# LIS-TU-Berlin/SVN-ICP

Measured on AMD Instinct MI355X. Metric: scan-pair registrations/sec at N particles x M source pts, 1/2/4/8 GPU, higher is better.
Workload: dtype f64; 1 GPU; C3: 128 particles SVN-ICP, 131072-pt source vs 262144-pt target, K=100, I=20, max_dist=1.0, lr=1.0, SVNFullGrad=False, correspondence=fast, early stop off; synthetic 64-beam scans (seed 20250718); particles=128, target_points=262144, knn_count=100, parallelism=single GPU

## Files before the change

### __graft_entry__.py

```python
from __future__ import annotations

import importlib.util
import os
import subprocess
import sys

ROOT = os.path.dirname(os.path.abspath(__file__))
PKG_DIR = os.path.join(ROOT, "svn-icp_amd")


def load_package():
    if "svnicp_amd" in sys.modules:
        return sys.modules["svnicp_amd"]
    spec = importlib.util.spec_from_file_location("svnicp_amd", os.path.join(PKG_DIR, "__init__.py"),
                                                  submodule_search_locations=[PKG_DIR])
    mod = importlib.util.module_from_spec(spec)
    sys.modules["svnicp_amd"] = mod
    spec.loader.exec_module(mod)
    return mod


def load_oracle():
    if "oracle_py" in sys.modules:
        return sys.modules["oracle_py"]
    spec = importlib.util.spec_from_file_location("oracle_py", os.path.join(ROOT, "oracle", "oracle_py.py"))
    mod = importlib.util.module_from_spec(spec)
    sys.modules["oracle_py"] = mod
    spec.loader.exec_module(mod)
    return mod


def build() -> None:
    jobs = str(min(4, os.cpu_count() or 1))
    subprocess.check_call(["make", "-C", os.path.join(PKG_DIR, "csrc"), "-j", jobs])
    subprocess.check_call(["make", "-C", os.path.join(ROOT, "oracle"), "libsvnicp_oracle.so"])
    subprocess.check_call(["make", "-C", os.path.join(ROOT, "tests", "microbench")])
    if os.path.isdir("/root/reference"):
        subprocess.check_call(["make", "-C", os.path.join(ROOT, "oracle"), "ref"])
    build_cpp_host()
    pkg = load_package()
    pkg.load_library()


def build_cpp_host() -> str:
    host = os.path.join(PKG_DIR, "host")
    exe = os.path.join(host, "sharded_drive")
    srcs = [os.path.join(host, f) for f in ("sharded_drive.cpp", "sharded_registration.hpp", "svnicp_hip_shim.hpp")]
    srcs.append(os.path.join(PKG_DIR, "libsvnicp_hip.so"))
    if os.path.exists(exe) and all(os.path.getmtime(exe) >= os.path.getmtime(f) for f in srcs):
        return exe
    subprocess.check_call(["/opt/rocm/bin/hipcc", "-std=c++17", "-O2", "-Wall", "-Werror", "-I", os.path.join(ROOT, "include"), "-I", host,
                           os.path.join(host, "sharded_drive.cpp"), "-L", PKG_DIR, "-lsvnicp_hip", "-lrccl",
                           "-Wl,-rpath,$ORIGIN/..", "-o", exe])
    return exe


def smoke() -> None:
    import numpy as np
    pkg = load_package()
    orc = load_oracle()
    P, B, M, K, I = 8, 512, 2048, 16, 6
    src, tgt = pkg.scans.random_clouds(B, M, seed=3)
    init = pkg.scans.make_particles(P, seed=3) * 0.2
    prm = pkg.SteinICPParam(iterations=I, lr=1.0, max_dist=1.0, KNN_count=K, SVN_full_grad=False)
    s = pkg.SVNICP(prm, init, pkg.ParticleWeightOpt())
    s.add_cloud(src, tgt, init)
    s.set_initial_mean(np.eye(4))
    assert s.stein_align() == pkg.SteinICPState.ALIGN_SUCCESS
    o = orc.Solver(init, iterations=I, lr=1.0, max_dist=1.0, knn_count=K, svn_full_grad=False)
    o.add_cloud(src, tgt, init)
    o.stein_align()
    assert np.array_equal(s.get_candidates().astype(np.int64), o.candidates()), "stage-A indices differ from oracle"
    err = np.abs(s.get_transformation() - o.get_transformation()).max()
    assert err < 1e-4, f"pose differs from oracle by {err}"
    print(f"smoke ok: pose {s.get_transformation()}  |hip - oracle|max = {err:.3e}")


if __name__ == "__main__":
    build()
    if len(sys.argv) > 1 and sys.argv[1] == "smoke":
        smoke()
```

### svn-icp_amd/csrc/api.hip

```cpp
#include "../../include/svnicp_hip.h"

#include <cmath>
#include <algorithm>
#include <cstdio>
#include <cstdlib>
#include <cstring>
#include <string>
#include <vector>

#include "device_buffer.hpp"
#include "kernels.hpp"
#include "stage_a_host.hpp"
#include "stage_b_host.hpp"

using namespace svnicp;
using namespace svnicp_host;

namespace {

struct CloudState {
  DevBuf<double> src, tgt;
  bool src_set = false, tgt_set = false;
};

struct SteinState {
  DevBuf<double> init_pose, R, t, Rtot, pose_out, eul, opt, uctl, work, stats;
  DevBuf<float> history;
  DevBuf<int> ctl;
  int hist_I = 0, hist_P = 0;
  PinnedBuf<double> h_init, h_stats;
  bool host_stats_valid = false;
  Event ev_init;
  bool init_in_flight = false;
  StepPlan step;
  DrivePlan drive;
  int single_done_it = -1;
  Event ev_fork, ev_join;
  bool median_pending = false;
  DevBuf<unsigned int> small_bar;
  bool small_launched = false;
  Event ev_chunk[3];
  PinnedBuf<int> h_flags;
  bool finish_seen = true;
  int finish_iter = 0;
};

struct Sharding {
  int p_lo = 0, p_hi = 0;
  bool set = false;
  int row_rank = 0, row_world = 1;
  int64_t B_total = 0;
  DevBuf<double> rank_sums;
};

struct MiniBatch {
  int batch = 0;
  uint64_t seed = 0, n = 0;
  bool explicit_tab = false;
  int tab_I = 0;
  std::vector<int32_t> tab_h;
  int64_t tab_checked_B = -1;
  bool on = false, have = false;
  bool check = false;
  int64_t rows = 0, nq = 0;
  unsigned long long base = 0;
  DevBuf<int32_t> tab, idx, flag, pos, bsum, cand;
  DevBuf<int> ctl;
  DevBuf<double> src_u, src;
};

struct PlaneState {
  int residual = SVNICP_RESIDUAL_POINT;
  double delta = 0.1;
  int normal_k = 16;
  bool supplied = false;
  bool estimated = false;
  int est_k = 0;
  int64_t passes = 0;
  bool on = false;
  DevBuf<double> rec;
  DevBuf<double> nsup;
  DevBuf<int32_t> nbr;
  DevBuf<double> nbr_d2;
  DevBuf<double> partial, Hb, stats;
};

struct EvalState {
  DevBuf<double> q, d2, partial, result;
  DevBuf<int32_t> idx;
  PinnedBuf<double> h_result;
  bool have = false;
  int64_t rows = 0;
};

struct ScoreState {
  int kind = SVNICP_WEIGHT_UNIFORM;
  double gate = 0.0, temperature = 0.0;
  bool on = false;
  const char* reg_refusal = nullptr;
  DevBuf<double> partial, scores, poses, w;
  bool have = false;
  int P = 0;
};

struct Trace { DevBuf<double> H, b, N, phi, h; DevBuf<int32_t> corr; };

struct Profiling {
  Event ev[3];
  bool on = false;
  unsigned mask = 0;
  int pcur = -1;
  std::vector<Event> pev;
  std::vector<int> pcls;
  size_t pused = 0;
};

struct DebugCounters {
  DevBuf<unsigned long long> upd;
};

struct Progress {
  bool particles_set = false, began = false, have_candidates = false, have_result = false;
  bool table_built = false;
  bool d2_due = false;
};

}

struct svnicp_ctx {
  svnicp_params prm{};
  int device = 0, num_cus = 256;
  Stream own_stream, side;
  hipStream_t stream = nullptr;
  std::string err;
  static std::string& create_error() { thread_local std::string s; return s; }

  int64_t B = 0, M = 0;
  int K = 0, P = 0;
  Pose0 pose0{};
  Tuning tune{};
  CloudState cloud; StageA sa; StageB sb; SteinState st;
  Sharding shard; MiniBatch mb; PlaneState pl; EvalState ev; ScoreState sc;
  Trace tr; Profiling prof; DebugCounters dbg; Progress run;
};

enum { KC_KNN = 0, KC_TABLE = 1, KC_SEARCH = 2, KC_ACCUM = 3, KC_REDUCE = 4, KC_UPDATE = 5, KC_COUNT = SVNICP_KERNEL_CLASSES };

static hipError_t prof_begin(svnicp_ctx* c, int cls) {
  c->prof.pcur = -1;
  if (!c->prof.on || !((c->prof.mask >> cls) & 1u)) return hipSuccess;
  c->prof.pcur = cls;
  if (c->prof.pused * 2 + 2 > c->prof.pev.size()) {
    for (int i = 0; i < 2; ++i) {
      Event e;
      hipError_t r = e.create();
      if (r != hipSuccess) return r;
      c->prof.pev.push_back(std::move(e));
    }
    c->prof.pcls.push_back(cls);
  }
  c->prof.pcls[c->prof.pused] = cls;
  return hipEventRecord(c->prof.pev[2 * c->prof.pused], c->stream);
}
static hipError_t prof_end(svnicp_ctx* c) {
  if (!c->prof.on || c->prof.pcur < 0) return hipSuccess;
  c->prof.pcur = -1;
  hipError_t r = hipEventRecord(c->prof.pev[2 * c->prof.pused + 1], c->stream);
  c->prof.pused += 1;
  return r;
}

#define CTX_CHECK(ctx) do { if (!(ctx)) return SVNICP_ERR_INVALID; } while (0)

static int bind(svnicp_ctx* c) {
  HIPCHK(c, hipSetDevice(c->device));
  return 0;
}

static StageAEnv stage_a_env(const svnicp_ctx* c) {
  return {c->stream, c->tune, c->num_cus, c->prm.record_trace != 0, c->cloud.tgt.p, c->B, c->M, c->pose0};
}

static RegistrationFacts registration_facts(const svnicp_ctx* c, bool plane) {
  RegistrationFacts f;
  f.P = c->P; f.K = c->K; f.I = c->prm.iterations; f.B = c->B; f.M = c->M;
  f.svgd = c->prm.mode == SVNICP_MODE_SVGD; f.check_early_stop = c->prm.check_early_stop != 0; f.record_trace = c->prm.record_trace != 0;
  f.profiling = c->prof.on;
  f.shard_set = c->shard.set; f.p_lo = c->shard.p_lo; f.p_hi = c->shard.p_hi; f.row_world = c->shard.row_world;
  f.batch = c->mb.batch; f.explicit_tab = c->mb.explicit_tab; f.tab_I = c->mb.tab_I;
  f.plane = plane; f.normals_supplied = c->pl.supplied; f.normal_k = c->pl.normal_k;
  f.weighting = c->sc.kind;
  return f;
}

extern "C" {

int svnicp_abi_version(void) { return SVNICP_ABI_VERSION; }

const char* svnicp_last_error(const svnicp_ctx* ctx) { return ctx ? ctx->err.c_str() : svnicp_ctx::create_error().c_str(); }

int svnicp_create(const svnicp_params* params, int device, const double* init_pose6xP, int P, svnicp_ctx** out) {
  if (!params || !out) return fail<svnicp_ctx>(nullptr, SVNICP_ERR_INVALID, "svnicp_create: null argument");
  if (params->struct_size != (int32_t)sizeof(svnicp_params))
    return fail<svnicp_ctx>(nullptr, SVNICP_ERR_INVALID, "svnicp_create: svnicp_params.struct_size mismatch");
  if (params->iterations < 0 || params->knn_count < 1)
    return fail<svnicp_ctx>(nullptr, SVNICP_ERR_INVALID, "svnicp_create: iterations >= 0 and knn_count >= 1 required");
  if (params->mode != SVNICP_MODE_SVN && params->mode != SVNICP_MODE_SVGD)
    return fail<svnicp_ctx>(nullptr, SVNICP_ERR_INVALID, "svnicp_create: unknown mode");
  int ndev = 0;
  if (hipGetDeviceCount(&ndev) != hipSuccess || ndev <= 0)
    return fail<svnicp_ctx>(nullptr, SVNICP_ERR_NO_DEVICE, "svnicp_create: no HIP device visible (this library has no CPU path)");
  if (device < 0 || device >= ndev) return fail<svnicp_ctx>(nullptr, SVNICP_ERR_INVALID, "svnicp_create: bad device ordinal");
  hipDeviceProp_t prop;
  if (hipSetDevice(device) != hipSuccess || hipGetDeviceProperties(&prop, device) != hipSuccess)
    return fail<svnicp_ctx>(nullptr, SVNICP_ERR_HIP, "svnicp_create: hipGetDeviceProperties failed");
  if (std::strncmp(prop.gcnArchName, "gfx950", 6) != 0)
    return fail<svnicp_ctx>(nullptr, SVNICP_ERR_NO_DEVICE,
                std::string("svnicp_create: device is ") + prop.gcnArchName + ", this library carries gfx950 code only");
  svnicp_ctx* c = new svnicp_ctx();
  c->prm = *params;
  c->device = device;
  c->num_cus = prop.multiProcessorCount > 0 ? prop.multiProcessorCount : 256;
  c->K = params->knn_count;
  c->st.finish_iter = params->iterations;
  const double I3[9] = {1, 0, 0, 0, 1, 0, 0, 0, 1};
  std::memcpy(c->pose0.R0, I3, sizeof I3);
  c->pose0.t0[0] = c->pose0.t0[1] = c->pose0.t0[2] = 0.0;
  if (c->own_stream.create(hipStreamNonBlocking) != hipSuccess) { delete c; return fail<svnicp_ctx>(nullptr, SVNICP_ERR_HIP, "svnicp_create: hipStreamCreate failed"); }
  if (c->side.create(hipStreamNonBlocking) != hipSuccess ||
      c->st.ev_fork.create(hipEventDisableTiming) != hipSuccess || c->st.ev_join.create(hipEventDisableTiming) != hipSuccess ||
      c->st.ev_init.create(hipEventDisableTiming) != hipSuccess) {
    delete c;
    return fail<svnicp_ctx>(nullptr, SVNICP_ERR_HIP, "svnicp_create: hipStreamCreate / hipEventCreate failed");
  }
  c->stream = c->own_stream;
  for (auto& e : c->prof.ev)
    if (e.create() != hipSuccess) { delete c; return fail<svnicp_ctx>(nullptr, SVNICP_ERR_HIP, "hipEventCreate failed"); }
  if (c->st.ctl.ensure(4) != hipSuccess) { delete c; return fail<svnicp_ctx>(nullptr, SVNICP_ERR_NOMEM, "hipMalloc failed"); }
  *out = c;
  if (const char* e = getenv("SVNICP_OPTIONS")) {
    std::string all(e);
    size_t pos = 0;
    while (pos < all.size()) {
      const size_t end = all.find(';', pos) == std::string::npos ? all.size() : all.find(';', pos);
      const std::string kv = all.substr(pos, end - pos);
      const size_t eq = kv.find('=');
      if (eq != std::string::npos && svnicp_set_option(c, kv.substr(0, eq).c_str(), kv.substr(eq + 1).c_str()) != 0) {
        svnicp_ctx::create_error() = c->err; svnicp_destroy(c); *out = nullptr; return SVNICP_ERR_INVALID;
      }
      pos = end + 1;
    }
  }
  if (init_pose6xP) {
    int rc = svnicp_set_particles(c, init_pose6xP, P);
    if (rc != 0) { svnicp_ctx::create_error() = c->err; svnicp_destroy(c); *out = nullptr; return rc; }
  }
  return SVNICP_OK;
}

void svnicp_destroy(svnicp_ctx* c) {
  if (!c) return;
  (void)hipSetDevice(c->device);
  if (c->stream) (void)hipStreamSynchronize(c->stream);
  if (c->side) (void)hipStreamSynchronize(c->side);
  delete c;
}

int svnicp_set_stream(svnicp_ctx* c, void* hip_stream) {
  CTX_CHECK(c);
  if (bind(c)) return SVNICP_ERR_HIP;
  HIPCHK(c, hipStreamSynchronize(c->stream));
  c->stream = hip_stream == SVNICP_OWN_STREAM ? c->own_stream : reinterpret_cast<hipStream_t>(hip_stream);
  return SVNICP_OK;
}

static int check_small_kernel(svnicp_ctx* c);
static int check_minibatch_table(svnicp_ctx* c);
int svnicp_synchronize(svnicp_ctx* c) {
  CTX_CHECK(c);
  if (bind(c)) return SVNICP_ERR_HIP;
  HIPCHK(c, hipStreamSynchronize(c->stream));
  if (const int rc = check_small_kernel(c)) return rc;
  if (const int rc = check_minibatch_table(c)) return rc;
  if (c->run.have_result && c->st.h_stats.p) c->st.host_stats_valid = true;
  return SVNICP_OK;
}

static int upload_cloud(svnicp_ctx* c, DevBuf<double>& buf, const double* xyz, int64_t n, int mem_kind) {
  if (bind(c)) return SVNICP_ERR_HIP;
  HIPCHK(c, buf.ensure((size_t)n * 3));
  const hipMemcpyKind kind = mem_kind == SVNICP_MEM_DEVICE ? hipMemcpyDeviceToDevice : hipMemcpyHostToDevice;
  HIPCHK(c, hipMemcpyAsync(buf.p, xyz, (size_t)n * 24, kind, c->stream));
  if (mem_kind != SVNICP_MEM_DEVICE) HIPCHK(c, hipStreamSynchronize(c->stream));
  c->run.have_candidates = false;
  return SVNICP_OK;
}

int svnicp_set_source(svnicp_ctx* c, const double* src, int64_t B, int mem_kind) {
  CTX_CHECK(c);
  if (!src || B < 1) return fail(c, SVNICP_ERR_INVALID, "svnicp_set_source: need B >= 1");
  if (B > 0x7fffffffLL) return fail(c, SVNICP_ERR_INVALID, "svnicp_set_source: cloud too large");
  if (const int rc = upload_cloud(c, c->cloud.src, src, B, mem_kind)) return rc;
  c->B = B;
  c->cloud.src_set = true;
  return SVNICP_OK;
}

int svnicp_set_target(svnicp_ctx* c, const double* tgt, int64_t M, int mem_kind) {
  CTX_CHECK(c);
  if (!tgt || M < 1) return fail(c, SVNICP_ERR_INVALID, "svnicp_set_target: need M >= 1");
  if (M > 0x7fffffffLL) return fail(c, SVNICP_ERR_INVALID, "svnicp_set_target: cloud too large");
  if (const int rc = upload_cloud(c, c->cloud.tgt, tgt, M, mem_kind)) return rc;
  c->M = M;
  c->sa.held = TargetLayout::None;
  c->cloud.tgt_set = true;
  c->pl.supplied = false; c->pl.estimated = false;
  return SVNICP_OK;
}

int svnicp_set_clouds(svnicp_ctx* c, const double* src, int64_t B, const double* tgt, int64_t M, int mem_kind) {
  CTX_CHECK(c);
  if (!src || !tgt || B < 1 || M < 1) return fail(c, SVNICP_ERR_INVALID, "svnicp_set_clouds: need B >= 1, M >= 1");
  if (M > 0x7fffffffLL || B > 0x7fffffffLL) return fail(c, SVNICP_ERR_INVALID, "svnicp_set_clouds: cloud too large");
  if (const int rc = svnicp_set_source(c, src, B, mem_kind)) return rc;
  return svnicp_set_target(c, tgt, M, mem_kind);
}

int svnicp_set_particles(svnicp_ctx* c, const double* init, int P) {
  CTX_CHECK(c);
  if (!init || P < 1) return fail(c, SVNICP_ERR_INVALID, "svnicp_set_particles: need P >= 1");
  if (bind(c)) return SVNICP_ERR_HIP;
  HIPCHK(c, c->st.init_pose.ensure((size_t)P * 6));
  HIPCHK(c, c->st.R.ensure((size_t)P * 9));
  HIPCHK(c, c->st.t.ensure((size_t)P * 3));
  HIPCHK(c, c->st.Rtot.ensure((size_t)P * 12));
  HIPCHK(c, c->st.pose_out.ensure((size_t)P * 6));
  HIPCHK(c, c->sb.sums.ensure((size_t)P * kNSums));
  HIPCHK(c, c->st.stats.ensure((size_t)48 + P));
  HIPCHK(c, c->st.work.ensure(update_workspace_doubles(P)));
  HIPCHK(c, c->st.eul.ensure((size_t)P * 6));
  HIPCHK(c, c->st.opt.ensure((size_t)P * 18));
  HIPCHK(c, c->st.uctl.ensure(update_uctl_doubles(P)));
  if ((size_t)P * 6 > c->st.h_init.cap || (size_t)P + 48 > c->st.h_stats.cap) {
    HIPCHK(c, hipStreamSynchronize(c->stream));
    HIPCHK(c, c->st.h_init.alloc((size_t)P * 6));
    HIPCHK(c, c->st.h_stats.alloc((size_t)P + 48));
  } else if (c->st.init_in_flight) {
    HIPCHK(c, hipEventSynchronize(c->st.ev_init));
  }
  std::memcpy(c->st.h_init.p, init, (size_t)P * 48);
  HIPCHK(c, hipMemcpyAsync(c->st.init_pose.p, c->st.h_init.p, (size_t)P * 48, hipMemcpyHostToDevice, c->stream));
  HIPCHK(c, hipEventRecord(c->st.ev_init, c->stream));
  c->st.init_in_flight = true;
  c->st.host_stats_valid = false;
  const bool first = !c->run.particles_set || P != c->P;
  if (P != c->P) c->sc.have = false;
  if (first && c->shard.row_world > 1) { c->shard.row_world = 1; c->shard.row_rank = 0; c->shard.B_total = 0; }
  c->P = P;
  if (!c->shard.set || first) { c->shard.p_lo = 0; c->shard.p_hi = P; c->shard.set = false; }
  HIPCHK(c, launch_init_particles(c->st.init_pose.p, P, c->pose0, c->prm.mode, c->st.R.p, c->st.t.p, c->st.Rtot.p, c->st.pose_out.p,
                                  (first || c->prm.mode == SVNICP_MODE_SVN) ? 1 : 0, c->st.eul.p, c->stream));
  c->run.particles_set = true;
  return SVNICP_OK;
}

int svnicp_set_initial_mean(svnicp_ctx* c, const double R0[9], const double t0[3]) {
  CTX_CHECK(c);
  if (!R0 || !t0) return fail(c, SVNICP_ERR_INVALID, "svnicp_set_initial_mean: null argument");
  std::memcpy(c->pose0.R0, R0, 9 * sizeof(double));
  std::memcpy(c->pose0.t0, t0, 3 * sizeof(double));
  c->run.have_candidates = false;
  return SVNICP_OK;
}

int svnicp_set_k(svnicp_ctx* c, int k) {
  CTX_CHECK(c);
  if (k < 1) return fail(c, SVNICP_ERR_INVALID, "svnicp_set_k: k >= 1 required");
  c->K = k;
  c->run.have_candidates = false;
  return SVNICP_OK;
}

int svnicp_set_max_dist(svnicp_ctx* c, double md) {
  CTX_CHECK(c);
  c->prm.max_dist = md;
  return SVNICP_OK;
}

int svnicp_set_option(svnicp_ctx* c, const char* name, const char* value) {
  CTX_CHECK(c);
  if (!name || !value) return fail(c, SVNICP_ERR_INVALID, "svnicp_set_option: null argument");
  const std::string k(name), v(value);
  Tuning& t = c->tune;
  auto num = [&](int lo, int hi, int* out) { char* end = nullptr; const long x = strtol(v.c_str(), &end, 10);
                                             if (end == v.c_str() || *end || x < lo || x > hi) return false; *out = (int)x; return true; };
  bool ok = true;
  if (k == "knn") { if (v == "auto") t.knn = {}; else if (v == "v1") t.knn = {false, KnnKernel::Stream}; else if (v == "v2") t.knn = {false, KnnKernel::SeededScan};
                    else if (v == "brute") t.knn = {false, KnnKernel::Brute}; else if (v == "tiles") t.knn = {false, KnnKernel::Tiles}; else ok = false; }
  else if (k == "knn_prefilter") { if (v == "mfma") t.knn_prefilter_mfma = 1; else if (v == "valu") t.knn_prefilter_mfma = 0; else ok = false; }
  else if (k == "fallback_sliced_max") ok = num(-1, 1 << 20, &t.fallback_sliced_max);
  else if (k == "accum") { if (v == "f64") t.accum = 0; else if (v == "valu") t.accum = 1; else if (v == "split") t.accum = 3; else ok = false; }
  else if (k == "update") { if (v == "auto") t.update_fused = 0; else if (v == "fused") t.update_fused = 1; else ok = false; }
  else if (k == "fused_update_max_p") ok = num(1, 700, &t.fused_update_max_p);
  else if (k == "wgpcu") { int x = 0, y = 0; ok = sscanf(v.c_str(), "%d,%d", &x, &y) == 2 && x >= 0 && x <= 64 && y >= 0 && y <= 16; if (ok) { t.wgpcu_search = x; t.wgpcu_accum = y; } }
  else if (k == "tp") ok = num(0, 1 << 16, &t.tp);
  else if (k == "debug") ok = num(0, 1, &t.debug);
  else if (k == "scan_split") ok = num(0, 16, &t.scan_split);
  else if (k == "group_stride") ok = num(0, 1 << 30, &t.group_stride);
  else if (k == "accum_min_steps") ok = num(0, 1 << 20, &t.accum_min_steps);
  else if (k == "brute_qb") { ok = num(0, 6, &t.brute_qb); }
  else if (k == "single") { if (v == "fused") t.single_fused = 1; else if (v == "split") t.single_fused = 0; else ok = false; }
  else if (k == "chain") { if (v == "auto") { t.small_chain = 1; t.persistent = 0; } else if (v == "persistent") { t.small_chain = 1; t.persistent = 1; }
                           else if (v == "general") { t.small_chain = 0; t.persistent = 0; } else ok = false; }
  else if (k == "median") { if (v == "auto") t.median_inline = -1; else if (v == "stream") t.median_inline = 0; else if (v == "inline") t.median_inline = 1; else ok = false; }
  else if (k == "sort") { if (v == "joint") t.sort_joint = 1; else if (v == "separate") t.sort_joint = 0; else ok = false; }
  else if (k == "table") { if (v == "select") t.table_select = 1; else if (v == "gather") t.table_select = 0; else ok = false; }
  else if (k == "correspondence") { if (v == "fast") t.full_corr = 0; else if (v == "full") t.full_corr = 1; else ok = false; }
  else return fail(c, SVNICP_ERR_INVALID, "svnicp_set_option: unknown option '" + k + "'");
  if (!ok) return fail(c, SVNICP_ERR_INVALID, "svnicp_set_option: bad value '" + v + "' for option '" + k + "'");
  c->run.have_candidates = false;
  c->sa.held = TargetLayout::None;
  if (c->run.began) c->st.step = plan_step(registration_facts(c, c->pl.on), c->tune, c->sb.plan);
  return SVNICP_OK;
}

int svnicp_set_shard(svnicp_ctx* c, int p_lo, int p_hi) {
  CTX_CHECK(c);
  if (!c->run.particles_set || p_lo < 0 || p_hi > c->P || p_lo > p_hi)
    return fail(c, SVNICP_ERR_INVALID, "svnicp_set_shard: need 0 <= p_lo <= p_hi <= P after svnicp_set_particles");
  c->shard.p_lo = p_lo; c->shard.p_hi = p_hi; c->shard.set = true;
  return SVNICP_OK;
}

int svnicp_set_row_shard(svnicp_ctx* c, int row_rank, int row_world, int64_t total_source_points) {
  CTX_CHECK(c);
  if (!c->run.particles_set || row_world < 1 || row_rank < 0 || row_rank >= row_world || (row_world > 1 && total_source_points < 1))
    return fail(c, SVNICP_ERR_INVALID, "svnicp_set_row_shard: need 0 <= row_rank < row_world and the whole scan's point count, after svnicp_set_particles");
  if (bind(c)) return SVNICP_ERR_HIP;
  c->shard.row_rank = row_rank; c->shard.row_world = row_world;
  c->shard.B_total = row_world > 1 ? total_source_points : 0;
  if (row_world > 1) {
    HIPCHK(c, c->shard.rank_sums.ensure((size_t)row_world * c->P * kNSums));
    HIPCHK(c, hipMemsetAsync(c->shard.rank_sums.p, 0, (size_t)row_world * c->P * kNSums * sizeof(double), c->stream));
  }
  return SVNICP_OK;
}

void* svnicp_rank_sums_devptr(svnicp_ctx* c) { return (c && c->shard.row_world > 1) ? (void*)c->shard.rank_sums.p : nullptr; }

static bool normal_pass_due(const svnicp_ctx* c) {
  return c->pl.on && !c->pl.supplied && !(c->pl.estimated && c->pl.est_k == c->pl.normal_k);
}

static int prepare_plane(svnicp_ctx* c);
int svnicp_align_begin(svnicp_ctx* c) {
  CTX_CHECK(c);
  if (!c->cloud.src_set || !c->cloud.tgt_set || !c->run.particles_set)
    return fail(c, SVNICP_ERR_INVALID, "svnicp_align: svnicp_set_clouds and svnicp_set_particles must come first");
  if (bind(c)) return SVNICP_ERR_HIP;
  const int I = c->prm.iterations, P = c->P;
  const int64_t B = c->B;
  const bool plane = c->pl.residual == SVNICP_RESIDUAL_PLANE;
  const RegistrationFacts f = registration_facts(c, plane);
  if (const char* why = minibatch_refusal(f, c->tune)) return fail(c, SVNICP_ERR_INVALID, std::string(kMinibatchRefusal) + why);
  if (c->mb.batch != 0 && c->mb.explicit_tab && !c->mb.tab_h.empty() && c->mb.tab_checked_B != B) {
    for (const int32_t v : c->mb.tab_h)
      if (v < 0 || (int64_t)v >= B)
        return fail(c, SVNICP_ERR_INVALID, "svnicp_align: the mini-batch index table holds " + std::to_string(v) + ", outside [0, " + std::to_string(B) + ")");
    c->mb.tab_checked_B = B;
  }
  if (const char* why = plane_refusal(f, c->tune)) return fail(c, SVNICP_ERR_INVALID, std::string(kPlaneRefusal) + why);
  if (const char* why = weighting_refusal(f, c->tune)) return fail(c, SVNICP_ERR_INVALID, std::string(kWeightingRefusal) + why);
  if (f.weighting && score_tile_rows(P, c->K, true) < 1)
    return fail(c, SVNICP_ERR_INVALID, std::string(kWeightingRefusal) + "knn_count is too large for one row's candidates to fit the scoring kernel's LDS tile");
  const RegistrationRows r = registration_rows(c->mb.batch, I, B);
  const AccumPlan shape = plan_stage_b(f, c->tune, r.Bi);
  const bool stage_a_k1 = StageA::plan_for(stage_a_env(c), r.Bq, c->K).can_search(1);
  if (const char* why = full_corr_refusal(f, c->tune, shape.f32, stage_a_k1)) return fail(c, SVNICP_ERR_INVALID, why);
  c->pl.on = plane;
  c->sc.on = f.weighting != 0; c->sc.reg_refusal = scoring_refusal(f, c->tune);
  c->mb.on = r.mb; c->mb.have = false; c->mb.check = false;
  c->mb.rows = r.mb ? r.Bt : 0;
  c->mb.nq = r.mb ? r.Bq : 0;
  HIPCHK(c, hipEventRecord(c->prof.ev[0], c->stream));
  const bool joint = joint_morton_sort(f, c->tune, StageA::plan_for(stage_a_env(c), r.Bq, c->K));
  if (const int rc = c->sa.begin(c, stage_a_env(c), r.Bq, c->K, {c->K, normal_pass_due(c) ? c->pl.normal_k : c->K, c->tune.full_corr ? 1 : c->K}, joint)) return rc;
  c->sa.writes_table = select_writes_table(f, c->tune, c->sa.plan, shape);
  c->run.table_built = false; c->run.d2_due = false;
  if (r.mb) {
    HIPCHK(c, c->mb.idx.ensure((size_t)r.Bt)); HIPCHK(c, c->mb.flag.ensure((size_t)B)); HIPCHK(c, c->mb.pos.ensure((size_t)B));
    HIPCHK(c, c->mb.bsum.ensure((size_t)minibatch_scan_blocks(B))); HIPCHK(c, c->mb.ctl.ensure(2));
    HIPCHK(c, c->mb.src_u.ensure((size_t)r.Bq * 3)); HIPCHK(c, c->mb.src.ensure((size_t)r.Bt * 3));
    HIPCHK(c, c->mb.cand.ensure((size_t)r.Bt * c->K));
  }
  if (const int rc = c->sb.begin(c, f, c->tune, r, shape, c->num_cus)) return rc;
  HIPCHK(c, c->st.history.ensure((size_t)(I > 0 ? I : 1) * 6 * P));
  c->st.hist_I = I; c->st.hist_P = P;
  if (c->prm.record_trace) {
    const size_t IP = (size_t)I * P;
    HIPCHK(c, c->tr.corr.ensure(IP * r.Bi));
    HIPCHK(c, hipMemsetAsync(c->tr.corr.p, 0xff, IP * r.Bi * 4, c->stream));
    const struct { DevBuf<double>& buf; size_t n; } dbl[] = {{c->tr.H, IP * 36}, {c->tr.b, IP * 6}, {c->tr.N, IP * 6}, {c->tr.phi, IP * 6}, {c->tr.h, (size_t)I + 1}};
    for (const auto& x : dbl) {
      HIPCHK(c, x.buf.ensure(x.n));
      HIPCHK(c, hipMemsetAsync(x.buf.p, 0, x.n * 8, c->stream));
    }
  }
  c->prof.pused = 0;
  c->st.single_done_it = -1;
  if (c->st.median_pending) HIPCHK(c, hipStreamWaitEvent(c->stream, c->st.ev_join, 0));
  c->st.median_pending = false;
  if (!c->st.finish_seen && c->prm.mode == SVNICP_MODE_SVGD && c->prm.check_early_stop) {
    int v[2] = {0, 0};
    HIPCHK(c, hipMemcpyAsync(v, c->st.ctl.p, sizeof v, hipMemcpyDeviceToHost, c->stream));
    HIPCHK(c, hipStreamSynchronize(c->stream));
    if (v[0]) c->st.finish_iter = v[1];
    c->st.finish_seen = true;
  }
  {
    BeginZero z{};
    auto add = [&](void* p, size_t bytes) { if (p && bytes) { z.ptr[z.n] = static_cast<unsigned int*>(p); z.dwords[z.n] = (unsigned int)(bytes / 4); ++z.n; } };
    add(c->st.uctl.p, update_uctl_doubles(P) * sizeof(double));
    add(c->st.history.p, (size_t)(I > 0 ? I : 1) * 6 * P * sizeof(float));
    add(c->sb.ambig.p, 2 * sizeof(int));
    if (c->sa.plan.kernel == KnnKernel::Brute) add(c->sa.fail_count.p, sizeof(int));
    HIPCHK(c, c->st.small_bar.ensure(8));
    add(c->st.small_bar.p, 8 * sizeof(unsigned int));
    if (c->prm.mode == SVNICP_MODE_SVGD) add(c->st.opt.p, (size_t)P * 18 * sizeof(double));
    z.ctl = c->st.ctl.p; z.iterations = I;
    HIPCHK(c, launch_init_particles(c->st.init_pose.p, P, c->pose0, 2, c->st.R.p, c->st.t.p, c->st.Rtot.p, c->st.pose_out.p, 0,
                                    nullptr, c->stream, &z));
  }
  if (c->mb.batch > 0 && !c->mb.explicit_tab) {
    c->mb.base = minibatch_stream_base(c->mb.seed, c->mb.n);
    c->mb.n += 1;
  }
  if (plane)
    if (const int rc = prepare_plane(c)) return rc;
  c->st.step = plan_step(f, c->tune, c->sb.plan);
  c->run.began = true;
  c->st.finish_seen = false;
  c->run.have_result = false;
  return SVNICP_OK;
}

static int ensure_dbg_upd(svnicp_ctx* c) {
  if (!c->tune.debug || c->dbg.upd.p) return SVNICP_OK;
  HIPCHK(c, c->dbg.upd.ensure(8));
  HIPCHK(c, hipMemset(c->dbg.upd.p, 0, 8 * sizeof(unsigned long long)));
  return SVNICP_OK;
}

static int print_update_phases(svnicp_ctx* c, bool persistent) {
  unsigned long long h[8];
  HIPCHK(c, hipStreamSynchronize(c->stream));
  if (!persistent) HIPCHK(c, hipStreamSynchronize(c->side));
  HIPCHK(c, hipMemcpy(h, c->dbg.upd.p, sizeof h, hipMemcpyDeviceToHost));
  if (persistent)
    fprintf(stderr, "[svnicp] k_small_registration, workgroup 0, cycles over %d iterations: search %llu | barrier %llu | accumulate %llu | barrier %llu | prepare %llu | barrier %llu | direction %llu | barrier %llu\n",
            c->prm.iterations, h[0], h[1], h[2], h[3], h[4], h[5], h[6], h[7]);
  else
    fprintf(stderr, "[svnicp] Stein step thread-0 cycles (summed over launches so far; fused kernel: prepare / median / direction / pose / tail; k_upd_median: state / histogram / bin scan / collect / rank): %llu %llu %llu %llu %llu\n", h[0], h[1], h[2], h[3], h[4]);
  return SVNICP_OK;
}

static int prepare_plane(svnicp_ctx* c) {
  HIPCHK(c, c->pl.partial.ensure((size_t)c->sb.plan.grid_x * c->sb.plan.Ppad * kPlaneSums));
  HIPCHK(c, c->pl.Hb.ensure((size_t)c->P * 42));
  HIPCHK(c, c->pl.stats.ensure((size_t)c->P * 2));
  HIPCHK(c, hipMemsetAsync(c->pl.stats.p, 0, (size_t)c->P * 2 * sizeof(double), c->stream));
  const int kn = c->pl.normal_k;
  if (!normal_pass_due(c)) return SVNICP_OK;
  if (!c->sa.plan.can_search(kn))
    return fail(c, SVNICP_ERR_INVALID, "svnicp_align: the seeded-scan stage A (option knn=v2, or a target beyond the tile kernel's range) cannot "
                                       "search with normal_k neighbours: supply the normals (svnicp_set_target_normals)");
  const int64_t M = c->M, rows = c->sa.block_rows(M);
  HIPCHK(c, c->pl.rec.ensure((size_t)M * 6));
  HIPCHK(c, c->pl.nbr.ensure((size_t)rows * kn));
  HIPCHK(c, c->pl.nbr_d2.ensure((size_t)rows * kn));
  const int rc = c->sa.search_blocks(c, stage_a_env(c), c->cloud.tgt.p, M, kn, c->pl.nbr.p, c->pl.nbr_d2.p, 0, [&](int64_t lo, int64_t n) {
    HIPCHK(c, launch_target_normals(c->cloud.tgt.p, M, c->pl.nbr.p, lo, n, kn, c->pl.rec.p, c->stream));
    return (int)SVNICP_OK;
  });
  if (rc) return rc;
  c->pl.estimated = true; c->pl.est_k = kn;
  c->pl.passes += 1;
  return SVNICP_OK;
}

int svnicp_stage_candidates(svnicp_ctx* c, int64_t b_lo, int64_t b_hi) {
  CTX_CHECK(c);
  if (!c->run.began) return fail(c, SVNICP_ERR_INVALID, "svnicp_stage_candidates: call svnicp_align_begin first");
  if (b_lo < 0 || b_hi > c->B || b_lo > b_hi) return fail(c, SVNICP_ERR_INVALID, "svnicp_stage_candidates: bad row range");
  if (bind(c)) return SVNICP_ERR_HIP;
  if (c->mb.on) {
    if (b_lo != 0 || b_hi != c->B)
      return fail(c, SVNICP_ERR_INVALID, "svnicp_stage_candidates: in mini-batch mode only the whole range (0, B) is accepted");
    MinibatchArgs m{};
    m.explicit_idx = c->mb.explicit_tab ? c->mb.tab.p : nullptr; m.idx = c->mb.idx.p; m.n = c->mb.rows; m.B = c->B; m.base = c->mb.base;
    m.flag = c->mb.flag.p; m.pos = c->mb.pos.p; m.block_sums = c->mb.bsum.p; m.mbctl = c->mb.ctl.p; m.ctl = c->st.ctl.p;
    m.src = c->cloud.src.p; m.src_u = c->mb.src_u.p; m.n_q = c->mb.nq;
    HIPCHK(c, prof_begin(c, KC_KNN));
    HIPCHK(c, launch_minibatch_draw_compact(m, c->stream));
    const int rc = c->sa.search(c, stage_a_env(c), c->mb.src_u.p, c->pose0, c->K, c->sa.cand_idx.p, c->sa.cand_d2.p, 0, c->mb.nq);
    if (rc) return rc;
    HIPCHK(c, launch_minibatch_expand(m, c->sa.cand_idx.p, c->K, c->mb.src.p, c->mb.cand.p, c->stream));
    HIPCHK(c, prof_end(c));
    c->mb.have = true;
    c->mb.check = c->mb.explicit_tab && c->mb.tab_h.empty();
    return SVNICP_OK;
  }
  HIPCHK(c, prof_begin(c, KC_KNN));
  const bool whole = b_lo == 0 && b_hi == c->B;
  const bool hand_over = c->sa.writes_table && whole;
  const TableOut tbl{c->sb.tablea.p, c->sb.anchor.p, c->sb.cmaxb.p};
  if (const int rc = c->sa.search(c, stage_a_env(c), c->cloud.src.p, c->pose0, c->K, c->sa.cand_idx.p, c->sa.cand_d2.p, b_lo, b_hi,
                                  hand_over ? &tbl : nullptr, whole)) return rc;
  c->run.table_built = hand_over; c->run.d2_due = hand_over;
  if (c->tune.full_corr)
    if (const int rc = c->sa.keep_stage_fallbacks(c, stage_a_env(c))) return rc;
  HIPCHK(c, prof_end(c));
  return SVNICP_OK;
}


int svnicp_build_candidate_table(svnicp_ctx* c) {
  CTX_CHECK(c);
  if (!c->run.began) return fail(c, SVNICP_ERR_INVALID, "svnicp_build_candidate_table: call svnicp_align_begin first");
  if (bind(c)) return SVNICP_ERR_HIP;
  if (c->mb.on && !c->mb.have) return fail(c, SVNICP_ERR_INVALID, "svnicp_build_candidate_table: call svnicp_stage_candidates(0, B) first");
  HIPCHK(c, prof_begin(c, KC_TABLE));
  const int32_t* cand = c->mb.on ? c->mb.cand.p : c->sa.cand_idx.p;
  const int64_t rows = c->mb.on ? c->mb.rows : c->B;
  if (!c->run.table_built)
    if (const int rc = c->sb.build_table(c, cand, rows, c->K, c->cloud.tgt.p, c->M, c->stream)) return rc;
  HIPCHK(c, prof_end(c));
  HIPCHK(c, hipEventRecord(c->prof.ev[1], c->stream));
  c->run.have_candidates = true;
  return SVNICP_OK;
}

static UpdateArgs update_args(svnicp_ctx* c, int it) {
  UpdateArgs u{};
  u.sums = c->shard.row_world > 1 ? c->shard.rank_sums.p : c->sb.sums.p; u.n_ranks = c->shard.row_world; u.R = c->st.R.p; u.t = c->st.t.p; u.Rtot = c->st.Rtot.p; u.pose = c->pose0;
  u.P = c->P; u.iteration = it; u.iterations = c->prm.iterations;
  u.lr = c->prm.lr; u.conv_thr = c->prm.convergence_threshold;
  u.check_early_stop = c->prm.check_early_stop; u.full_grad = c->prm.svn_full_grad;
  u.work = c->st.work.p; u.history = c->st.history.p; u.pose_out = c->st.pose_out.p; u.ctl = c->st.ctl.p;
  if (c->prm.record_trace) {
    u.trH = c->tr.H.p + (size_t)it * c->P * 36; u.trb = c->tr.b.p + (size_t)it * c->P * 6;
    u.trN = c->tr.N.p + (size_t)it * c->P * 6; u.trphi = c->tr.phi.p + (size_t)it * c->P * 6; u.trh = c->tr.h.p + it;
  }
  u.eul = c->st.eul.p; u.opt = c->st.opt.p; u.optimizer = c->prm.optimizer;
  u.n_src = (double)(c->shard.row_world > 1 ? c->shard.B_total : c->B);
  u.uctl = c->st.uctl.p;
  u.dbg = c->tune.debug ? c->dbg.upd.p : nullptr;
  u.svgd = c->prm.mode == SVNICP_MODE_SVGD ? 1 : 0;
  u.plane_Hb = c->pl.on ? c->pl.Hb.p : nullptr;
  return u;
}
static AccumArgs accum_args(svnicp_ctx* c, int it) {
  AccumArgs a{};
  a.src = c->cloud.src.p; a.table = c->sb.table.p; a.tablef = c->sb.tablef.p; a.tablea = c->sb.tablea.p; a.kbest = c->sb.kbest.p; a.kidx = c->sb.kidx.p; a.tgt = c->cloud.tgt.p; a.cand = c->sa.cand_idx.p; a.anchor = c->sb.anchor.p; a.M = c->M; a.cmax = c->sb.cmaxb.p; a.ambig_count = c->sb.ambig.p;
  a.Rtot = c->st.Rtot.p; a.B = c->B; a.K = c->K;
  a.p_lo = c->shard.p_lo; a.p_hi = c->shard.p_hi; a.max_dist = c->prm.max_dist; a.partial = c->sb.partial.p; a.ctl = c->st.ctl.p;
  a.corr = c->prm.record_trace ? c->tr.corr.p + (size_t)it * c->P * c->B : nullptr;
  if (c->mb.on) {
    const size_t r0 = (size_t)it * c->mb.batch;
    a.src = c->mb.src.p + 3 * r0; a.cand = c->mb.cand.p + r0 * c->K; a.cmax = c->sb.cmaxb.p + r0; a.B = c->mb.batch;
    if (c->sb.table.p) a.table = c->sb.table.p + r0 * c->K * 3;
    if (c->sb.tablef.p) a.tablef = c->sb.tablef.p + r0 * c->K;
    if (c->sb.tablea.p) a.tablea = c->sb.tablea.p + r0 * 128;
    if (c->sb.anchor.p) a.anchor = c->sb.anchor.p + 3 * r0;
    if (c->prm.record_trace) a.corr = c->tr.corr.p + (size_t)it * c->P * c->mb.batch;
  }
  a.svgd = c->prm.mode == SVNICP_MODE_SVGD ? 1 : 0;
  a.fin_iteration = -1;
  if (c->st.drive.defer_fin && it >= 1) {
    const UpdateArgs up = update_args(c, it - 1);
    a.fin_iteration = it - 1; a.fin_P = c->P; a.fin_thr = c->prm.convergence_threshold; a.fin_norms = update_step_norms(up);
    a.fin_pose = c->st.pose_out.p; a.fin_history = c->st.history.p; a.fin_ctl = c->st.ctl.p;
  }
  a.ticket = reinterpret_cast<unsigned int*>(c->st.uctl.p + 41);
  return a;
}

static bool step_finishes(const svnicp_ctx* c, int it) { return !(c->st.drive.defer_fin && it < c->prm.iterations - 1); }

static int fork_median(svnicp_ctx* c, int it) {
  if (c->st.step.chain != StepChain::SideStream || c->st.median_pending) return SVNICP_OK;
  if (const int rc = ensure_dbg_upd(c)) return rc;
  const UpdateArgs u = update_args(c, it);
  HIPCHK(c, hipEventRecord(c->st.ev_fork, c->stream));
  HIPCHK(c, hipStreamWaitEvent(c->side, c->st.ev_fork, 0));
  HIPCHK(c, launch_update_median(u, c->num_cus, c->tune.fused_update_max_p, c->side));
  HIPCHK(c, hipEventRecord(c->st.ev_join, c->side));
  c->st.median_pending = true;
  return SVNICP_OK;
}

int svnicp_iter_accumulate(svnicp_ctx* c, int it) {
  CTX_CHECK(c);
  if (!c->run.began || !c->run.have_candidates)
    return fail(c, SVNICP_ERR_INVALID, "svnicp_iter_accumulate: candidates not staged");
  if (it < 0 || it >= c->prm.iterations) return fail(c, SVNICP_ERR_INVALID, "svnicp_iter_accumulate: bad iteration");
  if (bind(c)) return SVNICP_ERR_HIP;
  if (const int rc = fork_median(c, it)) return rc;
  const int nshard = c->shard.p_hi - c->shard.p_lo;
  if (nshard <= 0) return SVNICP_OK;
  AccumArgs a = accum_args(c, it);
  if (c->tune.full_corr) {
    HIPCHK(c, prof_begin(c, KC_SEARCH));
    for (int p = c->shard.p_lo; p < c->shard.p_hi; ++p) {
      HIPCHK(c, launch_transform_cloud(c->cloud.src.p, c->B, c->st.Rtot.p + 12 * (size_t)p, c->sb.full_q.p, c->st.ctl.p, c->stream));
      if (const int rc = c->sa.search_blocks(c, stage_a_env(c), c->sb.full_q.p, c->B, 1, c->sb.full_idx.p + (size_t)p * c->B, c->sb.full_d2.p, 1)) return rc;
    }
    HIPCHK(c, prof_end(c));
    a.full_idx = c->sb.full_idx.p;
  } else if (c->sb.plan.f32 == 3) {
    HIPCHK(c, prof_begin(c, KC_SEARCH));
    HIPCHK(c, launch_search_split(c->sb.plan, a, c->stream));
    HIPCHK(c, prof_end(c));
  }
  if (c->pl.on) {
    PlaneArgs pa{};
    pa.src = c->cloud.src.p; pa.rec = c->pl.rec.p; pa.Rtot = c->st.Rtot.p; pa.B = c->B; pa.M = c->M; pa.p_lo = c->shard.p_lo; pa.p_hi = c->shard.p_hi;
    pa.max_dist = c->prm.max_dist; pa.delta = c->pl.delta; pa.partial = c->pl.partial.p; pa.ctl = c->st.ctl.p;
    pa.kidx = c->sb.kidx.p; pa.kbest = c->sb.kbest.p; pa.corr = a.corr;
    HIPCHK(c, prof_begin(c, KC_ACCUM));
    HIPCHK(c, launch_plane_accumulate(c->sb.plan, pa, c->stream));
    HIPCHK(c, prof_end(c));
    HIPCHK(c, prof_begin(c, KC_REDUCE));
    HIPCHK(c, launch_plane_finalize(c->pl.partial.p, c->sb.plan.grid_x, c->sb.plan.Ppad, c->shard.p_lo, nshard, c->pl.Hb.p, c->pl.stats.p,
                                    c->st.ctl.p, c->stream));
    HIPCHK(c, prof_end(c));
    return SVNICP_OK;
  }
  const bool single = c->st.step.single_fused;
  const UpdateArgs us = update_args(c, it);
  HIPCHK(c, prof_begin(c, KC_ACCUM));
  HIPCHK(c, launch_accumulate(c->sb.plan, a, single ? &us : nullptr, c->stream));
  HIPCHK(c, prof_end(c));
  if (single) { c->st.single_done_it = it; return SVNICP_OK; }
  if (c->st.step.chain == StepChain::SmallChain) return SVNICP_OK;
  HIPCHK(c, prof_begin(c, KC_REDUCE));
  double* rec = c->shard.row_world > 1 ? c->shard.rank_sums.p + (size_t)c->shard.row_rank * c->P * kNSums : c->sb.sums.p;
  HIPCHK(c, launch_reduce_partials(c->sb.partial.p, c->sb.plan.grid_x, c->sb.plan.Ppad, c->shard.p_lo, nshard, rec, c->st.ctl.p, c->stream));
  HIPCHK(c, prof_end(c));
  return SVNICP_OK;
}

int svnicp_iter_update(svnicp_ctx* c, int it) {
  CTX_CHECK(c);
  if (!c->run.began) return fail(c, SVNICP_ERR_INVALID, "svnicp_iter_update: call svnicp_align_begin first");
  if (it < 0 || it >= c->prm.iterations) return fail(c, SVNICP_ERR_INVALID, "svnicp_iter_update: bad iteration");
  if (bind(c)) return SVNICP_ERR_HIP;
  if (c->st.single_done_it == it) { c->st.single_done_it = -1; return SVNICP_OK; }
  if (const int rc = ensure_dbg_upd(c)) return rc;
  UpdateArgs u = update_args(c, it);
  HIPCHK(c, prof_begin(c, KC_UPDATE));
  if (c->tune.debug && it == c->prm.iterations - 1)
    if (const int rc = print_update_phases(c, false)) return rc;
  const StepChain chain = c->st.step.chain;
  if (chain == StepChain::OneKernel) {
    u.svgd = 0;
    if (c->prm.mode == SVNICP_MODE_SVGD) HIPCHK(c, launch_update_svgd(u, c->stream));
    else HIPCHK(c, launch_update(u, c->stream));
  } else {
    if (chain == StepChain::SmallChain) {
      u.sums = c->sb.partial.p; u.n_ranks = c->sb.plan.grid_x; u.sums_stride = c->sb.plan.Ppad * kNSums; u.sums_out = c->sb.sums.p;
    }
    if (chain == StepChain::SideStream) {
      if (const int rc = fork_median(c, it)) return rc;
      HIPCHK(c, launch_update_prepare(u, c->stream));
      HIPCHK(c, hipStreamWaitEvent(c->stream, c->st.ev_join, 0));
      c->st.median_pending = false;
    } else {
      HIPCHK(c, launch_update_prepare_median(u, c->stream));
    }
    HIPCHK(c, launch_update_direction(u, c->stream, step_finishes(c, it)));
  }
  HIPCHK(c, prof_end(c));
  return SVNICP_OK;
}

static int enqueue_scoring(svnicp_ctx* c, double gate) {
  const bool normals = c->pl.supplied || c->pl.estimated;
  if (score_tile_rows(c->P, c->K, normals) < 1)
    return fail(c, SVNICP_ERR_INVALID, std::string(kScoringRefusal) + "knn_count is too large for one row's candidates to fit the scoring kernel's LDS tile");
  ScoreState& sc = c->sc;
  sc.have = false;
  HIPCHK(c, sc.partial.ensure((size_t)score_blocks(c->B) * score_padded_particles(c->P, c->K) * kScoreRecord));
  HIPCHK(c, sc.scores.ensure((size_t)c->P * kScoreFields));
  HIPCHK(c, sc.poses.ensure((size_t)c->P * 12));
  ScoreArgs a{};
  a.src = c->cloud.src.p; a.tgt = c->cloud.tgt.p; a.rec = normals ? c->pl.rec.p : nullptr; a.cand = c->sa.cand_idx.p; a.Rtot = c->st.Rtot.p;
  a.B = c->B; a.M = c->M; a.K = c->K; a.P = c->P; a.thr2 = gate * gate; a.partial = sc.partial.p;
  HIPCHK(c, launch_particle_score(a, sc.scores.p, c->stream));
  HIPCHK(c, hipMemcpyAsync(sc.poses.p, c->st.Rtot.p, (size_t)c->P * 12 * sizeof(double), hipMemcpyDeviceToDevice, c->stream));
  sc.have = true; sc.P = c->P;
  return SVNICP_OK;
}

int svnicp_finish(svnicp_ctx* c) {
  CTX_CHECK(c);
  if (!c->run.began) return fail(c, SVNICP_ERR_INVALID, "svnicp_finish: call svnicp_align_begin first");
  if (bind(c)) return SVNICP_ERR_HIP;
  HIPCHK(c, hipEventRecord(c->prof.ev[2], c->stream));
  StatsArgs s{c->st.pose_out.p, c->P, c->prm.mode, c->st.stats.p};
  if (c->sc.on) {
    if (const int rc = enqueue_scoring(c, c->sc.gate)) return rc;
    HIPCHK(c, c->sc.w.ensure((size_t)c->P));
    HIPCHK(c, launch_particle_weights(c->sc.scores.p, c->P, c->sc.temperature, c->sc.w.p, c->stream));
    HIPCHK(c, launch_stats_weighted(s, c->sc.w.p, c->stream));
  } else {
    HIPCHK(c, launch_stats(s, c->stream));
  }
  c->st.host_stats_valid = false;
  if (c->st.h_stats.p && (size_t)c->P + 48 <= c->st.h_stats.cap)
    HIPCHK(c, hipMemcpyAsync(c->st.h_stats.p, c->st.stats.p, ((size_t)c->P + 48) * 8, hipMemcpyDeviceToHost, c->stream));
  c->run.have_result = true;
  return SVNICP_OK;
}

int svnicp_stopped(svnicp_ctx* c) {
  CTX_CHECK(c);
  if (bind(c)) return SVNICP_ERR_HIP;
  int v[2] = {0, 0};
  HIPCHK(c, hipMemcpyAsync(v, c->st.ctl.p, sizeof v, hipMemcpyDeviceToHost, c->stream));
  HIPCHK(c, hipStreamSynchronize(c->stream));
  return v[0] ? 1 : 0;
}

void* svnicp_candidates_devptr(svnicp_ctx* c) { return c ? (void*)c->sa.cand_idx.p : nullptr; }
void* svnicp_sums_devptr(svnicp_ctx* c) { return c ? (void*)c->sb.sums.p : nullptr; }
void* svnicp_total_pose_devptr(svnicp_ctx* c) { return c ? (void*)c->st.Rtot.p : nullptr; }

static int align_enqueue(svnicp_ctx* c, bool follow_stop) {
  CTX_CHECK(c);
  if (c->prm.mode == SVNICP_MODE_SVGD && (c->prm.optimizer < 0 || c->prm.optimizer > 3))
    return SVNICP_NO_OPTIMIZER;
  int rc = svnicp_align_begin(c);
  if (rc) return rc;
  if ((rc = svnicp_stage_candidates(c, 0, c->B))) return rc;
  if ((rc = svnicp_build_candidate_table(c))) return rc;
  c->st.small_launched = false;
  const DrivePlan drive = plan_drive(registration_facts(c, c->pl.on), c->tune, c->sb.plan, c->st.step, follow_stop);
  c->st.drive = drive;
  c->st.drive.defer_fin = false;
  if (drive.persistent_try) {
    const AccumArgs a = accum_args(c, 0);
    if ((rc = ensure_dbg_upd(c))) return rc;
    if (c->tune.debug) HIPCHK(c, hipMemsetAsync(c->dbg.upd.p, 0, 8 * sizeof(unsigned long long), c->stream));
    UpdateArgs u = update_args(c, 0);
    u.sums_out = c->sb.sums.p;
    const hipError_t e = launch_small_registration(c->sb.plan, a, u, c->prm.iterations, c->st.small_bar.p, c->num_cus, c->stream);
    if (e == hipSuccess && c->tune.debug)
      if ((rc = print_update_phases(c, true))) return rc;
    if (e == hipSuccess) { c->st.small_launched = true; return svnicp_finish(c); }
    (void)hipGetLastError();
  }
  c->st.drive.defer_fin = drive.defer_fin;
  struct Reset { bool& f; ~Reset() { f = false; } } reset_defer{c->st.drive.defer_fin};
  if (drive.follow && !c->st.h_flags.p) {
    HIPCHK(c, c->st.h_flags.alloc(3));
    for (auto& e : c->st.ev_chunk) HIPCHK(c, e.create(hipEventDisableTiming));
  }
  for (int it = 0; it < c->prm.iterations; ++it) {
    if ((rc = svnicp_iter_accumulate(c, it))) return rc;
    if ((rc = svnicp_iter_update(c, it))) return rc;
    if (drive.follow && (it + 1) % kChunk == 0) {
      const int chunk = it / kChunk, slot = chunk % 3;
      HIPCHK(c, hipMemcpyAsync(&c->st.h_flags.p[slot], c->st.ctl.p, sizeof(int), hipMemcpyDeviceToHost, c->stream));
      HIPCHK(c, hipEventRecord(c->st.ev_chunk[slot], c->stream));
      if (chunk >= 1) {
        const int prev = (chunk - 1) % 3;
        HIPCHK(c, hipEventSynchronize(c->st.ev_chunk[prev]));
        if (c->st.h_flags.p[prev]) break;
      }
    }
  }
  return svnicp_finish(c);
}
int svnicp_align_async(svnicp_ctx* c) { return align_enqueue(c, false); }

static int check_small_kernel(svnicp_ctx* c) {
  if (!c->st.small_launched) return SVNICP_OK;
  c->st.small_launched = false;
  unsigned int w[2] = {0u, 0u};
  HIPCHK(c, hipMemcpyAsync(w, c->st.small_bar.p, sizeof w, hipMemcpyDeviceToHost, c->stream));
  HIPCHK(c, hipStreamSynchronize(c->stream));
  if (w[1] != 0u) { c->run.have_result = false; return fail(c, SVNICP_ERR_HIP, "svnicp_align: the small-registration kernel's grid barrier timed out (chain=persistent is an option; the default launches do not wait on each other)"); }
  return SVNICP_OK;
}

static int check_minibatch_table(svnicp_ctx* c) {
  if (!c->mb.check) return SVNICP_OK;
  c->mb.check = false;
  int w[2] = {0, 0};
  HIPCHK(c, hipMemcpyAsync(w, c->mb.ctl.p, sizeof w, hipMemcpyDeviceToHost, c->stream));
  HIPCHK(c, hipStreamSynchronize(c->stream));
  if (w[0]) {
    c->run.have_result = false; c->st.finish_seen = true;
    return fail(c, SVNICP_ERR_INVALID, "svnicp_align: the mini-batch index table holds a value outside [0, B); the registration did not run");
  }
  return SVNICP_OK;
}

int svnicp_align(svnicp_ctx* c) {
  CTX_CHECK(c);
  if (c->shard.set && (c->shard.p_lo != 0 || c->shard.p_hi != c->P))
    return fail(c, SVNICP_ERR_INVALID, "svnicp_align: a particle shard is set; drive the split-phase calls instead");
  if (c->shard.row_world > 1)
    return fail(c, SVNICP_ERR_INVALID, "svnicp_align: a source-row shard is set (this context holds a partial record); drive the split-phase calls instead");
  int rc = align_enqueue(c, true);
  if (rc) return rc;
  HIPCHK(c, hipStreamSynchronize(c->stream));
  if ((rc = check_small_kernel(c))) return rc;
  if ((rc = check_minibatch_table(c))) return rc;
  c->st.host_stats_valid = c->st.h_stats.p != nullptr;
  return SVNICP_ALIGN_SUCCESS;
}

static int fetch(svnicp_ctx* c, void* dst, const void* src, size_t bytes) {
  if (bind(c)) return SVNICP_ERR_HIP;
  HIPCHK(c, hipMemcpyAsync(dst, src, bytes, hipMemcpyDeviceToHost, c->stream));
  HIPCHK(c, hipStreamSynchronize(c->stream));
  return SVNICP_OK;
}
#define NEED_RESULT(c)                                                                   \
  do {                                                                                   \
    CTX_CHECK(c);                                                                        \
    if (!(c)->run.have_result) return fail((c), SVNICP_ERR_INVALID, "no registration result yet"); \
  } while (0)

static int fetch_stats(svnicp_ctx* c, void* dst, size_t off_doubles, size_t n_doubles) {
  if (c->st.host_stats_valid) { std::memcpy(dst, c->st.h_stats.p + off_doubles, n_doubles * 8); return SVNICP_OK; }
  return fetch(c, dst, c->st.stats.p + off_doubles, n_doubles * 8);
}
int svnicp_get_transformation(svnicp_ctx* c, double out6[6]) { NEED_RESULT(c); return fetch_stats(c, out6, 0, 6); }
int svnicp_get_distribution(svnicp_ctx* c, double out6[6]) { NEED_RESULT(c); return fetch_stats(c, out6, 6, 6); }
int svnicp_get_cov_matrix(svnicp_ctx* c, double out36[36]) { NEED_RESULT(c); return fetch_stats(c, out36, 12, 36); }
int svnicp_get_particle_weight(svnicp_ctx* c, double* outP) {
  NEED_RESULT(c);
  return fetch_stats(c, outP, 48, (size_t)c->P);
}
int svnicp_get_particles(svnicp_ctx* c, double* out6P) {
  CTX_CHECK(c);
  if (!c->run.particles_set) return fail(c, SVNICP_ERR_INVALID, "no particles set");
  return fetch(c, out6P, c->st.pose_out.p, (size_t)c->P * 48);
}
int svnicp_get_particle_history(svnicp_ctx* c, float* out) {
  NEED_RESULT(c);
  return fetch(c, out, c->st.history.p, (size_t)c->st.hist_I * 6 * c->st.hist_P * sizeof(float));
}

int svnicp_get_gpu_ms(svnicp_ctx* c, double out3[3]) {
  NEED_RESULT(c);
  if (bind(c)) return SVNICP_ERR_HIP;
  HIPCHK(c, hipStreamSynchronize(c->stream));
  float a = 0, b = 0;
  HIPCHK(c, hipEventElapsedTime(&a, c->prof.ev[0], c->prof.ev[1]));
  HIPCHK(c, hipEventElapsedTime(&b, c->prof.ev[1], c->prof.ev[2]));
  out3[0] = a; out3[1] = b; out3[2] = (double)a + b;
  return SVNICP_OK;
}

int svnicp_get_runtime(svnicp_ctx* c, double out3[3]) {
  NEED_RESULT(c);
  double ms[3];
  int rc = svnicp_get_gpu_ms(c, ms);
  if (rc) return rc;
  if (c->prm.mode == SVNICP_MODE_SVGD && c->prm.check_early_stop && !c->st.finish_seen) {
    int v[2] = {0, 0};
    HIPCHK(c, hipMemcpy(v, c->st.ctl.p, sizeof v, hipMemcpyDeviceToHost));
    if (v[0]) c->st.finish_iter = v[1];
    c->st.finish_seen = true;
  }
  out3[0] = ms[0] * 1e-3; out3[1] = ms[1] * 1e-3; out3[2] = (double)c->st.finish_iter;
  return SVNICP_OK;
}

int svnicp_get_iterations_run(svnicp_ctx* c, int* out) {
  NEED_RESULT(c);
  if (!out) return SVNICP_ERR_INVALID;
  int v[2];
  const int rc = fetch(c, v, c->st.ctl.p, sizeof v);
  if (rc) return rc;
  *out = v[1];
  return SVNICP_OK;
}

int svnicp_get_knn_fallbacks(svnicp_ctx* c, int* out) {
  CTX_CHECK(c);
  if (!c->run.have_candidates) return fail(c, SVNICP_ERR_INVALID, "no candidates yet");
  const int* count = c->sa.fallback_count();
  if (!count) { *out = -1; return SVNICP_OK; }
  return fetch(c, out, count, sizeof(int));
}

int svnicp_get_knn_fallback_rows(svnicp_ctx* c, int32_t* out, int cap, int* n_out) {
  CTX_CHECK(c);
  if (!c->run.have_candidates || !n_out) return fail(c, SVNICP_ERR_INVALID, "no candidates yet");
  *n_out = 0;
  const int* count = c->sa.fallback_count();
  if (!count) return SVNICP_OK;
  int n = 0;
  int rc = fetch(c, &n, count, sizeof(int));
  if (rc) return rc;
  *n_out = n;
  if (n > cap) n = cap;
  if (n > 0 && out) return fetch(c, out, c->sa.fallback_rows(), (size_t)n * 4);
  return SVNICP_OK;
}

int svnicp_get_knn_survivors(svnicp_ctx* c, int32_t* outB) {
  CTX_CHECK(c);
  const int32_t* n = c->run.have_candidates ? c->sa.survivors(c->prm.record_trace != 0) : nullptr;
  if (!n) return fail(c, SVNICP_ERR_INVALID, "svnicp_get_knn_survivors: needs record_trace and the pruned stage-A kernel");
  return fetch(c, outB, n, (size_t)c->B * 4);
}

int svnicp_get_ambiguous_steps(svnicp_ctx* c, int* out) {
  NEED_RESULT(c);
  if (c->sb.plan.f32 == 0) { *out = -1; return SVNICP_OK; }
  return fetch(c, out, c->sb.ambig.p, sizeof(int));
}

int svnicp_get_ambiguous_pairs(svnicp_ctx* c, int64_t* out) {
  CTX_CHECK(c);
  if (!c->run.have_result || !out) return fail(c, SVNICP_ERR_INVALID, "no registration result yet");
  if (c->sb.plan.f32 != 3) { *out = -1; return SVNICP_OK; }
  int v[2] = {0, 0};
  const int rc = fetch(c, v, c->sb.ambig.p, sizeof v);
  *out = v[1];
  return rc;
}

int svnicp_set_profile(svnicp_ctx* c, int on) {
  CTX_CHECK(c);
  c->prof.on = on != 0;
  c->prof.mask = on == 1 ? ~0u : ((unsigned)on >> 1);
  return SVNICP_OK;
}

int svnicp_get_kernel_ms(svnicp_ctx* c, double* ms5, int32_t* launches5) {
  NEED_RESULT(c);
  if (!c->prof.on) return fail(c, SVNICP_ERR_INVALID, "svnicp_get_kernel_ms: profiling is off (svnicp_set_profile)");
  if (bind(c)) return SVNICP_ERR_HIP;
  HIPCHK(c, hipStreamSynchronize(c->stream));
  for (int i = 0; i < KC_COUNT; ++i) { ms5[i] = 0.0; launches5[i] = 0; }
  for (size_t i = 0; i < c->prof.pused; ++i) {
    float ms = 0;
    HIPCHK(c, hipEventElapsedTime(&ms, c->prof.pev[2 * i], c->prof.pev[2 * i + 1]));
    ms5[c->prof.pcls[i]] += ms;
    launches5[c->prof.pcls[i]] += 1;
  }
  return SVNICP_OK;
}

static const char* const kMbCandMsg = "mini-batch mode: stage A ran on the drawn rows only, use svnicp_get_minibatch_candidates";
int svnicp_get_candidates(svnicp_ctx* c, int32_t* out) {
  CTX_CHECK(c);
  if (!c->run.have_candidates) return fail(c, SVNICP_ERR_INVALID, "no candidates yet");
  if (c->mb.on) return fail(c, SVNICP_ERR_INVALID, std::string("svnicp_get_candidates: ") + kMbCandMsg);
  return fetch(c, out, c->sa.cand_idx.p, (size_t)c->B * c->K * 4);
}
int svnicp_get_candidate_dist2(svnicp_ctx* c, double* out) {
  CTX_CHECK(c);
  if (!c->run.have_candidates) return fail(c, SVNICP_ERR_INVALID, "no candidates yet");
  if (c->mb.on) return fail(c, SVNICP_ERR_INVALID, std::string("svnicp_get_candidate_dist2: ") + kMbCandMsg);
  if (c->run.d2_due) {
    if (bind(c)) return SVNICP_ERR_HIP;
    HIPCHK(c, launch_candidate_dist2(c->cloud.src.p, c->pose0, c->cloud.tgt.p, c->M, c->sa.cand_idx.p, c->B, c->K, c->sa.cand_d2.p, c->stream));
    c->run.d2_due = false;
  }
  return fetch(c, out, c->sa.cand_d2.p, (size_t)c->B * c->K * 8);
}

int svnicp_set_minibatch(svnicp_ctx* c, int batch_size, uint64_t seed) {
  CTX_CHECK(c);
  c->mb.batch = batch_size;
  c->mb.seed = seed; c->mb.n = 0;
  c->mb.explicit_tab = false; c->mb.tab_I = 0; c->mb.tab_h.clear(); c->mb.tab_checked_B = -1;
  c->run.have_candidates = false;
  return SVNICP_OK;
}

int svnicp_set_minibatch_indices(svnicp_ctx* c, const int32_t* idx, int iterations, int batch_size, int mem_kind) {
  CTX_CHECK(c);
  if (!idx || iterations < 1 || batch_size < 1)
    return fail(c, SVNICP_ERR_INVALID, "svnicp_set_minibatch_indices: need a table of iterations >= 1 rows of batch_size >= 1 indices");
  const int64_t n = (int64_t)iterations * batch_size;
  if (n > kMinibatchMaxRows) return fail(c, SVNICP_ERR_INVALID, "svnicp_set_minibatch_indices: iterations * batch_size exceeds 2^22 table rows");
  if (bind(c)) return SVNICP_ERR_HIP;
  HIPCHK(c, hipStreamSynchronize(c->stream));
  HIPCHK(c, c->mb.tab.ensure((size_t)n));
  c->mb.tab_h.clear();
  if (mem_kind == SVNICP_MEM_DEVICE) {
    HIPCHK(c, hipMemcpyAsync(c->mb.tab.p, idx, (size_t)n * 4, hipMemcpyDeviceToDevice, c->stream));
  } else {
    c->mb.tab_h.assign(idx, idx + n);
    HIPCHK(c, hipMemcpyAsync(c->mb.tab.p, c->mb.tab_h.data(), (size_t)n * 4, hipMemcpyHostToDevice, c->stream));
    HIPCHK(c, hipStreamSynchronize(c->stream));
  }
  c->mb.batch = batch_size; c->mb.explicit_tab = true; c->mb.tab_I = iterations; c->mb.tab_checked_B = -1;
  c->run.have_candidates = false;
  return SVNICP_OK;
}

#define NEED_MINIBATCH(c, what)                                                                                          \
  do {                                                                                                                   \
    CTX_CHECK(c);                                                                                                        \
    if (!(c)->mb.on || !(c)->mb.have) return fail((c), SVNICP_ERR_INVALID, what ": no registration in mini-batch mode yet"); \
  } while (0)
int svnicp_get_minibatch_indices(svnicp_ctx* c, int32_t* out) {
  NEED_MINIBATCH(c, "svnicp_get_minibatch_indices");
  return fetch(c, out, c->mb.idx.p, (size_t)c->mb.rows * 4);
}
int svnicp_get_minibatch_candidates(svnicp_ctx* c, int32_t* out) {
  NEED_MINIBATCH(c, "svnicp_get_minibatch_candidates");
  return fetch(c, out, c->mb.cand.p, (size_t)c->mb.rows * c->K * 4);
}
int svnicp_get_minibatch_rows(svnicp_ctx* c, int64_t out2[2]) {
  NEED_MINIBATCH(c, "svnicp_get_minibatch_rows");
  if (!out2) return SVNICP_ERR_INVALID;
  int w[2] = {0, 0};
  const int rc = fetch(c, w, c->mb.ctl.p, sizeof w);
  if (rc) return rc;
  out2[0] = w[1]; out2[1] = c->mb.nq;
  return SVNICP_OK;
}

int svnicp_set_residual(svnicp_ctx* c, int residual, double huber_delta, int normal_k) {
  CTX_CHECK(c);
  if (residual != SVNICP_RESIDUAL_POINT && residual != SVNICP_RESIDUAL_PLANE) return fail(c, SVNICP_ERR_INVALID, "svnicp_set_residual: unknown residual");
  if (!(huber_delta > 0.0)) return fail(c, SVNICP_ERR_INVALID, "svnicp_set_residual: huber_delta must be positive (+inf: no down-weighting)");
  if (normal_k != 0 && (normal_k < 4 || normal_k > 64)) return fail(c, SVNICP_ERR_INVALID, "svnicp_set_residual: normal_k must be 0 (= 16) or in 4..64");
  c->pl.residual = residual; c->pl.delta = huber_delta; c->pl.normal_k = normal_k ? normal_k : 16;
  c->run.have_candidates = false;
  return SVNICP_OK;
}

int svnicp_set_target_normals(svnicp_ctx* c, const double* n_xyz, int64_t M, int mem_kind) {
  CTX_CHECK(c);
  if (!n_xyz) return fail(c, SVNICP_ERR_INVALID, "svnicp_set_target_normals: null argument");
  if (!c->cloud.tgt_set || M != c->M)
    return fail(c, SVNICP_ERR_INVALID, "svnicp_set_target_normals: must follow the svnicp_set_target it belongs to, with the same point count");
  if (bind(c)) return SVNICP_ERR_HIP;
  HIPCHK(c, c->pl.nsup.ensure((size_t)M * 3));
  HIPCHK(c, c->pl.rec.ensure((size_t)M * 6));
  HIPCHK(c, hipMemcpyAsync(c->pl.nsup.p, n_xyz, (size_t)M * 24, mem_kind == SVNICP_MEM_DEVICE ? hipMemcpyDeviceToDevice : hipMemcpyHostToDevice, c->stream));
  HIPCHK(c, launch_pack_normals(c->cloud.tgt.p, c->pl.nsup.p, M, c->pl.rec.p, c->stream));
  if (mem_kind != SVNICP_MEM_DEVICE) HIPCHK(c, hipStreamSynchronize(c->stream));
  c->pl.supplied = true; c->pl.estimated = false;
  return SVNICP_OK;
}

int svnicp_get_target_normals(svnicp_ctx* c, double* outMx3) {
  CTX_CHECK(c);
  if (!outMx3) return fail(c, SVNICP_ERR_INVALID, "svnicp_get_target_normals: null argument");
  if (!c->pl.supplied && !c->pl.estimated) return fail(c, SVNICP_ERR_INVALID, "svnicp_get_target_normals: no normals supplied or estimated for this target yet");
  std::vector<double> rec((size_t)c->M * 6);
  if (const int rc = fetch(c, rec.data(), c->pl.rec.p, rec.size() * 8)) return rc;
  for (int64_t i = 0; i < c->M; ++i)
    for (int d = 0; d < 3; ++d) outMx3[3 * i + d] = rec[6 * i + 3 + d];
  return SVNICP_OK;
}

int svnicp_get_plane_stats(svnicp_ctx* c, double* outPx2, int64_t* normal_passes) {
  CTX_CHECK(c);
  if (normal_passes) *normal_passes = c->pl.passes;
  if (!outPx2) return SVNICP_OK;
  if (!c->run.have_result || !c->pl.on) return fail(c, SVNICP_ERR_INVALID, "svnicp_get_plane_stats: no registration with the point-to-plane residual yet");
  return fetch(c, outPx2, c->pl.stats.p, (size_t)c->P * 16);
}

static void host_so3_exp(const double w[3], double R[9]) {
  const double th = std::sqrt(w[0] * w[0] + w[1] * w[1] + w[2] * w[2]);
  const double K[9] = {0, -w[2], w[1], w[2], 0, -w[0], -w[1], w[0], 0};
  double K2[9];
  for (int i = 0; i < 3; ++i)
    for (int j = 0; j < 3; ++j) K2[3 * i + j] = K[3 * i] * K[j] + K[3 * i + 1] * K[3 + j] + K[3 * i + 2] * K[6 + j];
  const double a = th < 1e-10 ? 1.0 : std::sin(th) / th, b = th < 1e-10 ? 0.5 : (1.0 - std::cos(th)) / (th * th);
  for (int i = 0; i < 9; ++i) R[i] = (i % 4 == 0 ? 1.0 : 0.0) + a * K[i] + b * K2[i];
}

int svnicp_evaluate(svnicp_ctx* c, const double* R, const double* t, double max_corr_dist, svnicp_eval* out) {
  CTX_CHECK(c);
  if (!out) return fail(c, SVNICP_ERR_INVALID, "svnicp_evaluate: null result struct");
  if (out->struct_size != (int32_t)sizeof(svnicp_eval)) return fail(c, SVNICP_ERR_INVALID, "svnicp_evaluate: svnicp_eval.struct_size mismatch");
  if (!(max_corr_dist > 0.0)) return fail(c, SVNICP_ERR_INVALID, "svnicp_evaluate: max_corr_dist must be positive and not NaN (+inf: every evaluated row with a finite distance is an inlier)");
  if ((R == nullptr) != (t == nullptr)) return fail(c, SVNICP_ERR_INVALID, "svnicp_evaluate: R and t must both be given, or both be NULL (the last registration's result)");
  if (R) {
    bool finite = true;
    for (int i = 0; i < 9; ++i) finite = finite && std::isfinite(R[i]);
    for (int i = 0; i < 3; ++i) finite = finite && std::isfinite(t[i]);
    if (!finite) return fail(c, SVNICP_ERR_INVALID, "svnicp_evaluate: the pose holds a non-finite entry");
  }
  if (!c->run.have_result)
    return fail(c, SVNICP_ERR_INVALID, "svnicp_evaluate: no finished registration yet (stage A's target layout and scratch belong to one)");
  if (!c->run.have_candidates)
    return fail(c, SVNICP_ERR_INVALID, "svnicp_evaluate: the source, the target, the initial mean, K or an option changed since the last registration: "
                                       "register again first (stage A's target layout and scratch belong to that registration)");
  if (!c->sa.plan.can_search(1))
    return fail(c, SVNICP_ERR_INVALID, "svnicp_evaluate: the seeded-scan stage A (option knn=v2, or a target beyond the tile kernel's range) is built "
                                       "for knn_count neighbours and cannot search with K = 1");
  if (const int rc = svnicp_synchronize(c)) return rc;
  EvalPose T{};
  if (R) {
    std::memcpy(T.R, R, sizeof T.R); std::memcpy(T.t, t, sizeof T.t);
  } else {
    double mean[6], Rc[9];
    if (const int rc = fetch_stats(c, mean, 0, 6)) return rc;
    host_so3_exp(mean + 3, Rc);
    const double* R0 = c->pose0.R0;
    for (int i = 0; i < 3; ++i) {
      for (int j = 0; j < 3; ++j) T.R[3 * i + j] = R0[3 * i] * Rc[j] + R0[3 * i + 1] * Rc[3 + j] + R0[3 * i + 2] * Rc[6 + j];
      T.t[i] = (R0[3 * i] * mean[0] + R0[3 * i + 1] * mean[1] + R0[3 * i + 2] * mean[2]) + c->pose0.t0[i];
    }
    for (int i = 0; i < 12; ++i)
      if (!std::isfinite(i < 9 ? T.R[i] : T.t[i - 9])) return fail(c, SVNICP_ERR_INVALID, "svnicp_evaluate: the last registration's result pose is not finite");
  }
  const int64_t B = c->B, M = c->M, nblk = evaluate_blocks(B);
  EvalState& ev = c->ev;
  ev.have = false;
  HIPCHK(c, ev.q.ensure((size_t)B * 3)); HIPCHK(c, ev.idx.ensure((size_t)B)); HIPCHK(c, ev.d2.ensure((size_t)B));
  HIPCHK(c, ev.partial.ensure((size_t)nblk * kEvalRecord)); HIPCHK(c, ev.result.ensure(kEvalResult));
  if (!ev.h_result.p) HIPCHK(c, ev.h_result.alloc(kEvalResult));
  HIPCHK(c, launch_evaluate_transform(c->cloud.src.p, B, T, ev.q.p, c->stream));
  const StageAEnv env{c->stream, c->tune, c->num_cus, false, c->cloud.tgt.p, c->B, c->M, c->pose0};
  if (!c->sa.stage_kept)
    if (const int rc = c->sa.keep_stage_fallbacks(c, env)) return rc;
  if (const int rc = c->sa.search_blocks(c, env, ev.q.p, B, 1, ev.idx.p, ev.d2.p, 1)) return rc;
  const bool normals = c->pl.supplied || c->pl.estimated;
  EvalArgs a{};
  a.q = ev.q.p; a.tgt = c->cloud.tgt.p; a.rec = normals ? c->pl.rec.p : nullptr; a.B = B; a.M = M;
  a.thr2 = max_corr_dist * max_corr_dist; a.idx = ev.idx.p; a.d2 = ev.d2.p; a.partial = ev.partial.p;
  HIPCHK(c, launch_evaluate_pairs(a, ev.result.p, c->stream));
  HIPCHK(c, hipMemcpyAsync(ev.h_result.p, ev.result.p, kEvalResult * sizeof(double), hipMemcpyDeviceToHost, c->stream));
  HIPCHK(c, hipStreamSynchronize(c->stream));
  const double* r = ev.h_result.p;
  out->has_normals = normals ? 1 : 0;
  out->rows = B;
  out->evaluated = (int64_t)r[0]; out->inliers = (int64_t)r[1]; out->plane_inliers = (int64_t)r[2];
  out->sum_d2 = r[3]; out->sum_r2 = r[4]; out->fitness = r[5]; out->inlier_rmse = r[6]; out->plane_rmse = r[7];
  std::memcpy(out->R, T.R, sizeof T.R); std::memcpy(out->t, T.t, sizeof T.t);
  ev.have = true; ev.rows = B;
  return SVNICP_OK;
}

const int32_t* svnicp_eval_index_devptr(svnicp_ctx* c) { return (c && c->ev.have) ? c->ev.idx.p : nullptr; }
const double* svnicp_eval_dist2_devptr(svnicp_ctx* c) { return (c && c->ev.have) ? c->ev.d2.p : nullptr; }

int svnicp_get_eval_pairs(svnicp_ctx* c, int32_t* idxB, double* d2B) {
  CTX_CHECK(c);
  if (!c->ev.have) return fail(c, SVNICP_ERR_INVALID, "svnicp_get_eval_pairs: no svnicp_evaluate yet");
  if (idxB)
    if (const int rc = fetch(c, idxB, c->ev.idx.p, (size_t)c->ev.rows * 4)) return rc;
  if (d2B)
    if (const int rc = fetch(c, d2B, c->ev.d2.p, (size_t)c->ev.rows * 8)) return rc;
  return SVNICP_OK;
}

int svnicp_get_particle_scores(svnicp_ctx* c, double* outPx6, double* posesPx12) {
  CTX_CHECK(c);
  if (!c->sc.have) return fail(c, SVNICP_ERR_INVALID, "svnicp_get_particle_scores: no scoring yet (svnicp_score_particles, or a registration with svnicp_set_particle_weighting)");
  if (outPx6)
    if (const int rc = fetch(c, outPx6, c->sc.scores.p, (size_t)c->sc.P * kScoreFields * sizeof(double))) return rc;
  if (posesPx12)
    if (const int rc = fetch(c, posesPx12, c->sc.poses.p, (size_t)c->sc.P * 12 * sizeof(double))) return rc;
  return SVNICP_OK;
}

int svnicp_score_particles(svnicp_ctx* c, double max_corr_dist, double* outPx6, double* posesPx12) {
  CTX_CHECK(c);
  if (!(max_corr_dist > 0.0) || !std::isfinite(max_corr_dist))
    return fail(c, SVNICP_ERR_INVALID, "svnicp_score_particles: max_corr_dist must be finite and positive");
  if (!c->run.have_result)
    return fail(c, SVNICP_ERR_INVALID, "svnicp_score_particles: no finished registration yet (the candidate table belongs to one)");
  if (!c->run.have_candidates)
    return fail(c, SVNICP_ERR_INVALID, "svnicp_score_particles: the source, the target, the initial mean, K or an option changed since the last registration: "
                                       "register again first (the candidate table belongs to that registration)");
  if (c->sc.reg_refusal) return fail(c, SVNICP_ERR_INVALID, std::string(kScoringRefusal) + c->sc.reg_refusal);
  if (const int rc = svnicp_synchronize(c)) return rc;
  if (bind(c)) return SVNICP_ERR_HIP;
  if (const int rc = enqueue_scoring(c, max_corr_dist)) return rc;
  if (!outPx6 && !posesPx12) { HIPCHK(c, hipStreamSynchronize(c->stream)); return SVNICP_OK; }
  return svnicp_get_particle_scores(c, outPx6, posesPx12);
}

int svnicp_set_particle_weighting(svnicp_ctx* c, int kind, double max_corr_dist, double temperature) {
  CTX_CHECK(c);
  if (kind != SVNICP_WEIGHT_UNIFORM) {
    if (!(max_corr_dist > 0.0) || !std::isfinite(max_corr_dist))
      return fail(c, SVNICP_ERR_INVALID, "svnicp_set_particle_weighting: max_corr_dist must be finite and positive");
    if (!(temperature > 0.0) || !std::isfinite(temperature))
      return fail(c, SVNICP_ERR_INVALID, "svnicp_set_particle_weighting: temperature must be finite and positive");
  }
  c->sc.kind = kind;
  c->sc.gate = max_corr_dist; c->sc.temperature = temperature;
  return SVNICP_OK;
}

int svnicp_get_trace(svnicp_ctx* c, int32_t* corr, double* H, double* b, double* N, double* phi, double* h) {
  NEED_RESULT(c);
  if (!c->prm.record_trace) return fail(c, SVNICP_ERR_INVALID, "svnicp_get_trace: params.record_trace was 0");
  const size_t I = (size_t)c->prm.iterations, P = (size_t)c->P;
  int rc = 0;
  if (corr && (rc = fetch(c, corr, c->tr.corr.p, I * P * (size_t)(c->mb.on ? c->mb.batch : c->B) * 4))) return rc;
  if (H && (rc = fetch(c, H, c->tr.H.p, I * P * 36 * 8))) return rc;
  if (b && (rc = fetch(c, b, c->tr.b.p, I * P * 6 * 8))) return rc;
  if (N && (rc = fetch(c, N, c->tr.N.p, I * P * 6 * 8))) return rc;
  if (phi && (rc = fetch(c, phi, c->tr.phi.p, I * P * 6 * 8))) return rc;
  if (h && (rc = fetch(c, h, c->tr.h.p, I * 8))) return rc;
  return SVNICP_OK;
}

}
```

### svn-icp_amd/csrc/kernels.hpp

```cpp
#pragma once
#include "device_math.hpp"
#include "registration_plan.hpp"
#include "stage_a_plan.hpp"

namespace svnicp {

struct KnnArgs {
  const double* src;
  Pose0 pose;
  const double *tx, *ty, *tz;
  const int32_t* torig;
  int64_t M, Mp;
  int64_t b_lo, b_hi;
  int K, S;
  double* pool_d;
  int32_t* pool_i;
  int32_t* out_idx;
  double* out_d2;
  const int32_t* qlist;
  const int* qlist_count;
  int list_grid;
  int list_qw;
  int slices, slice_max_queries, merge_n;
  double* sl_d;
  int32_t* sl_i;
  const double* qthr;
};
hipError_t launch_knn_merge_slices(const KnnArgs& a, hipStream_t st);

struct KnnBruteArgs {
  const double* src;
  Pose0 pose;
  const double* tgt;
  int64_t M;
  int64_t b_lo, b_hi;
  int K;
  int32_t* out_idx;
  double* out_d2;
  unsigned long long* phase_cycles;
};
int knn_brute_queries_per_block(int64_t n, int num_cus);
hipError_t launch_knn_brute(const KnnBruteArgs& a, int num_cus, int queries_per_block, hipStream_t st);

struct KnnScanArgs {
  const double* src;
  Pose0 pose;
  const double *tx, *ty, *tz;
  const float *txf, *tyf, *tzf;
  const int32_t* torig;
  const unsigned long long* emax_bits;
  int64_t M, Mp, Ms;
  int64_t b_lo, b_hi;
  int K, S2, seed_rank;
  int32_t* pool;
  int32_t* out_idx;
  double* out_d2;
  int32_t* fail_list;
  int* fail_count;
};
hipError_t launch_targets_soa2(const double* tgt, int64_t M, int64_t Mp, double* tx, double* ty, double* tz,
                               float* txf, float* tyf, float* tzf, int32_t* torig, unsigned long long* emax_bits,
                               hipStream_t st);
hipError_t launch_knn_scan(const KnnScanArgs& a, hipStream_t st);
hipError_t launch_knn_topk(const KnnArgs& a, hipStream_t st);

struct KnnTilesArgs {
  const double* src;
  Pose0 pose;
  const int32_t* qorder;
  const double *tx, *ty, *tz;
  const float *txf, *tyf, *tzf;
  const int32_t* torig;
  const float* tile_box;
  const unsigned long long* emax_bits;
  const float4* tile_a;
  const float4* tile_o;
  int prefilter_mfma;
  int64_t M, Mp;
  int n_tiles;
  int64_t b_lo, b_hi;
  int K, S2;
  int32_t* pool;
  int32_t* arena;
  int32_t* chunk_tab;
  int arena_cap;
  int64_t tab_rows;
  int scan_split;
  unsigned int group_stride;
  int32_t* out_idx;
  double* out_d2;
  const double* tgt;
  float4* tbl_a;
  double* tbl_anchor;
  float* tbl_cmax;
  int32_t* fail_list;
  int* fail_count;
  int32_t* stat_n;
  unsigned long long* phase_cycles;
  void* qrec;
  double* fail_tau;
};
hipError_t launch_knn_tiles(const KnnTilesArgs& a, hipStream_t st);
hipError_t launch_candidate_dist2(const double* src, const Pose0& pose, const double* tgt, int64_t M, const int32_t* idx, int64_t B, int K,
                                  double* d2, hipStream_t st);
size_t sort_temp_bytes(size_t n, int key_bits);
hipError_t launch_bbox(const double* pts, int64_t n, unsigned long long* bbox, hipStream_t st);
hipError_t launch_morton_order(const double* pts, int64_t i0, int64_t n, int transform, const Pose0& pose,
                               const unsigned long long* bbox, unsigned int* keys_a, unsigned int* keys_b,
                               int32_t* vals_a, int32_t* order, void* temp, size_t temp_bytes, hipStream_t st);
hipError_t launch_morton_order_joint(const double* tgt, int64_t M, const double* qsrc, int64_t n, const Pose0& pose,
                                     const unsigned long long* bbox, unsigned int* keys_a, unsigned int* keys_b,
                                     int32_t* vals_a, int32_t* order, void* temp, size_t temp_bytes, hipStream_t st);
hipError_t launch_targets_sorted(const double* tgt, int64_t M, int64_t Mp, const int32_t* order, double* tx, double* ty,
                                 double* tz, float* txf, float* tyf, float* tzf, int32_t* torig, float* tile_box,
                                 unsigned long long* emax_bits, float4* tile_a, float4* tile_o, hipStream_t st);

struct AccumArgs {
  const double* src;
  const double* table;
  const float4* tablef;
  const float4* tablea;
  const float* cmax;
  int* ambig_count;
  const double* Rtot;
  int64_t B;
  int K, RS;
  int p_lo, p_hi;
  int TP;
  int tiles_per_block;
  int64_t n_tiles;
  int Ppad;
  double max_dist;
  double* partial;
  const int* ctl;
  int32_t* corr;
  int svgd;
  const double* tgt;
  const int32_t* cand;
  const double* anchor;
  int64_t M;
  uint8_t* kbest;
  int32_t* kidx;
  const int32_t* full_idx;
  int pts_per_block, spts_per_block;
  unsigned int* ticket;
  int fin_iteration, fin_P;
  double fin_thr;
  const double* fin_norms;
  const double* fin_pose;
  float* fin_history;
  int* fin_ctl;
};
AccumPlan plan_accumulate(AccumPlan shape, int64_t B, int num_cus, const Tuning& tune);
hipError_t launch_search_split(const AccumPlan& plan, AccumArgs a, hipStream_t st);
hipError_t launch_accumulate_split(const AccumPlan& plan, const AccumArgs& a, hipStream_t st);
void split_occupancy_blocks(int PW, int WP, int K, size_t smem, int* search, int* accum);
hipError_t launch_build_table3(const int32_t* idx, int64_t B, int K, const double* tgt, int64_t M, double* table,
                               double* anchor, float4* tablea, float* cmax, hipStream_t st);
hipError_t launch_build_table3_list(const int32_t* idx, const int32_t* list, const int* count, int64_t B, int K, const double* tgt,
                                    int64_t M, double* anchor, float4* tablea, float* cmax, hipStream_t st);
hipError_t launch_build_table2(const int32_t* idx, int64_t B, int K, const double* tgt, int64_t M, double* table,
                               float4* tablef, float* cmax, hipStream_t st);
hipError_t launch_transform_cloud(const double* src, int64_t B, const double* pose12, double* q, const int* ctl, hipStream_t st);
struct UpdateArgs {
  const double* sums;
  int n_ranks;
  int sums_stride;
  double* sums_out;
  double* R;
  double* t;
  double* Rtot;
  Pose0 pose;
  int P, iteration, iterations;
  double lr, conv_thr;
  int check_early_stop, full_grad;
  double* work;
  float* history;
  double* pose_out;
  int* ctl;
  double *trH, *trb, *trN, *trphi, *trh;
  int h_in_lds;
  double* eul;
  double* opt;
  int svgd;
  int optimizer;
  double n_src;
  double* uctl;
  unsigned long long* dbg;
  const double* plane_Hb;
};
size_t update_workspace_doubles(int P);
struct BeginZero { unsigned int* ptr[6]; unsigned int dwords[6]; int n; int* ctl; int iterations; };
hipError_t launch_init_particles(const double* init6xP, int P, const Pose0& pose, int mode, double* R, double* t,
                                 double* Rtot, double* pose_out, int refresh_pose, double* eul, hipStream_t st, const BeginZero* zero = nullptr);
int single_particle_grid(int64_t B);
hipError_t launch_accumulate(const AccumPlan& plan, AccumArgs a, const UpdateArgs* single, hipStream_t st);
hipError_t launch_update_svgd(const UpdateArgs& a, hipStream_t st);
hipError_t launch_update(const UpdateArgs& a, hipStream_t st);
hipError_t launch_update_median(const UpdateArgs& a, int num_cus, int max_p_one_workgroup, hipStream_t st);
hipError_t launch_update_prepare(const UpdateArgs& a, hipStream_t st);
hipError_t launch_update_prepare_median(const UpdateArgs& a, hipStream_t st);
hipError_t launch_small_registration(const AccumPlan& plan, AccumArgs a, const UpdateArgs& u, int iterations, unsigned int* bar,
                                     int num_cus, hipStream_t st);
hipError_t launch_update_direction(const UpdateArgs& a, hipStream_t st, bool finish = true);
const double* update_step_norms(const UpdateArgs& a);
hipError_t launch_reduce_partials(const double* partial, int nblk, int Ppad, int p_lo, int n_particles, double* sums, const int* ctl,
                                  hipStream_t st);
size_t update_uctl_doubles(int P);
constexpr int kPlaneSums = 29;
constexpr double kPlaneMinRatio = 0.01;
struct PlaneArgs {
  const double* src;
  const double* rec;
  const double* Rtot;
  int64_t B, M;
  int p_lo, p_hi;
  int Ppad;
  int pts_per_block;
  double max_dist, delta;
  double* partial;
  const int* ctl;
  const int32_t* kidx;
  const uint8_t* kbest;
  int32_t* corr;
};
hipError_t launch_target_normals(const double* tgt, int64_t M, const int32_t* nbr, int64_t row_lo, int64_t rows, int kn, double* rec,
                                 hipStream_t st);
hipError_t launch_pack_normals(const double* tgt, const double* nrm, int64_t M, double* rec, hipStream_t st);
hipError_t launch_plane_accumulate(const AccumPlan& plan, PlaneArgs a, hipStream_t st);
hipError_t launch_plane_finalize(const double* partial, int nblk, int Ppad, int p_lo, int n_particles, double* Hb, double* stats,
                                 const int* ctl, hipStream_t st);
constexpr int kEvalRecord = 5;
constexpr int kEvalResult = 8;
struct EvalPose { double R[9]; double t[3]; };
struct EvalArgs {
  const double* q;
  const double* tgt;
  const double* rec;
  int64_t B, M;
  double thr2;
  int32_t* idx;
  double* d2;
  double* partial;
};
int64_t evaluate_blocks(int64_t B);
hipError_t launch_evaluate_transform(const double* src, int64_t B, const EvalPose& T, double* q, hipStream_t st);
hipError_t launch_evaluate_pairs(const EvalArgs& a, double* result, hipStream_t st);
constexpr int kScoreRecord = 5;
constexpr int kScoreFields = 6;
constexpr int kScoreRowsPerBlock = 64;
struct ScoreArgs {
  const double* src;
  const double* tgt;
  const double* rec;
  const int32_t* cand;
  const double* Rtot;
  int64_t B, M;
  int K, P;
  int Ppad, TH;
  double thr2;
  double* partial;
};
int64_t score_blocks(int64_t B);
int score_padded_particles(int P, int K);
int score_tile_rows(int P, int K, bool normals);
hipError_t launch_particle_score(ScoreArgs a, double* scores, hipStream_t st);
hipError_t launch_particle_weights(const double* scores, int P, double temperature, double* w, hipStream_t st);

struct MinibatchArgs {
  const int32_t* explicit_idx;
  int32_t* idx;
  int64_t n, B;
  unsigned long long base;
  int32_t* flag;
  int32_t* pos;
  int32_t* block_sums;
  int* mbctl;
  int* ctl;
  const double* src;
  double* src_u;
  int64_t n_q;
};
unsigned long long minibatch_stream_base(unsigned long long seed, unsigned long long registration);
int64_t minibatch_scan_blocks(int64_t B);
hipError_t launch_minibatch_draw_compact(const MinibatchArgs& a, hipStream_t st);
hipError_t launch_minibatch_expand(const MinibatchArgs& a, const int32_t* cand_u, int K, double* src_mb, int32_t* cand_mb,
                                   hipStream_t st);

struct StatsArgs { const double* pose; int P; int mode; double* out;  };
hipError_t launch_stats(const StatsArgs& a, hipStream_t st);
hipError_t launch_stats_weighted(const StatsArgs& a, const double* w, hipStream_t st);

}
```

### svn-icp_amd/csrc/particle_state.hip

```cpp
#include "kernels.hpp"

namespace svnicp {

namespace {

__global__ void k_init_particles(const double* __restrict__ init, int P, Pose0 pose, int mode, double* R, double* t,
                                 double* Rtot, double* pose_out, int refresh_pose, double* eul, BeginZero z) {
  const int p = blockIdx.x * blockDim.x + threadIdx.x;
  for (int a = 0; a < z.n; ++a)
    for (unsigned int e = (unsigned int)p; e < z.dwords[a]; e += gridDim.x * blockDim.x) z.ptr[a][e] = 0u;
  if (z.ctl && p == 0) { z.ctl[0] = 0; z.ctl[1] = z.iterations; z.ctl[2] = 0; z.ctl[3] = 0; }
  if (p >= P) return;
  double r[3] = {0, 0, 0}, tv[3], Rm[9];
  if (mode == 2) {
    for (int i = 0; i < 9; ++i) Rm[i] = R[9 * p + i];
    for (int i = 0; i < 3; ++i) tv[i] = t[3 * p + i];
  } else {
    r[0] = init[3 * P + p]; r[1] = init[4 * P + p]; r[2] = init[5 * P + p];
    tv[0] = init[p]; tv[1] = init[P + p]; tv[2] = init[2 * P + p];
    if (mode == 0) so3_exp(r, Rm, nullptr); else euler_to_R(r[0], r[1], r[2], Rm);
    if (mode == 1 && eul) {
      for (int i = 0; i < 3; ++i) { eul[6 * p + i] = tv[i]; eul[6 * p + 3 + i] = r[i]; }
    }
  }
  double Rt[9], tt[3];
  mat3_mul(pose.R0, Rm, Rt);
  mat3_vec(pose.R0, tv, tt);
  for (int i = 0; i < 9; ++i) { R[9 * p + i] = Rm[i]; Rtot[12 * p + i] = Rt[i]; }
  for (int i = 0; i < 3; ++i) { t[3 * p + i] = tv[i]; Rtot[12 * p + 9 + i] = pose.t0[i] + tt[i]; }
  if (refresh_pose) {
    double lg[3];
    if (mode == 0) so3_log(Rm, lg); else { lg[0] = r[0]; lg[1] = r[1]; lg[2] = r[2]; }
    for (int i = 0; i < 3; ++i) { pose_out[i * P + p] = tv[i]; pose_out[(3 + i) * P + p] = lg[i]; }
  }
}

__global__ void k_stats(StatsArgs a) {
  const int tid = threadIdx.x;
  const int P = a.P;
  __shared__ double mean[6];
  constexpr int kStage = 1024;
  __shared__ double sp[6 * kStage];
  const bool staged = P <= kStage;
  if (staged) for (int e = tid; e < 6 * P; e += blockDim.x) sp[e] = a.pose[e];
  __syncthreads();
  const double* pose = staged ? sp : a.pose;
  const double wsvn = (double)(1.0f / (float)P);
  if (tid < 6) {
    double s = 0.0;
    if (a.mode == 0) { for (int p = 0; p < P; ++p) s += pose[tid * P + p] * wsvn; }
    else { for (int p = 0; p < P; ++p) s += pose[tid * P + p]; s /= P; }
    mean[tid] = s;
    a.out[tid] = s;
  }
  __syncthreads();
  if (tid < 6) {
    double s = 0.0;
    if (a.mode == 0) { for (int p = 0; p < P; ++p) { const double d = pose[tid * P + p] - mean[tid]; s += d * d * wsvn; } }
    else { for (int p = 0; p < P; ++p) { const double d = pose[tid * P + p] - mean[tid]; s += d * d; } s /= (P - 1); }
    a.out[6 + tid] = s;
  }
  if (tid < 36) {
    const int r = tid / 6, c = tid % 6;
    double s = 0.0;
    const double wgt = a.mode == 0 ? wsvn : 1.0;
    for (int p = 0; p < P; ++p) s += wgt * ((pose[r * P + p] - mean[r]) * (pose[c * P + p] - mean[c]));
    a.out[12 + tid] = a.mode == 0 ? s : s / P;
  }
  for (int p = tid; p < P; p += blockDim.x) a.out[48 + p] = a.mode == 0 ? wsvn : 1.0;
}

__global__ void k_stats_weighted(StatsArgs a, const double* __restrict__ w) {
  const int tid = threadIdx.x;
  const int P = a.P;
  __shared__ double mean[6];
  constexpr int kStage = 896;
  __shared__ double sp[7 * kStage];
  const bool staged = P <= kStage;
  if (staged) {
    for (int e = tid; e < 6 * P; e += blockDim.x) sp[e] = a.pose[e];
    for (int e = tid; e < P; e += blockDim.x) sp[6 * P + e] = w[e];
  }
  __syncthreads();
  const double* pose = staged ? sp : a.pose;
  const double* wp = staged ? sp + 6 * P : w;
  if (tid < 6) {
    double s = 0.0;
    for (int p = 0; p < P; ++p) s += pose[tid * P + p] * wp[p];
    mean[tid] = s;
    a.out[tid] = s;
  }
  __syncthreads();
  if (tid < 6) {
    double s = 0.0;
    for (int p = 0; p < P; ++p) { const double d = pose[tid * P + p] - mean[tid]; s += d * d * wp[p]; }
    a.out[6 + tid] = s;
  }
  if (tid < 36) {
    const int r = tid / 6, c = tid % 6;
    double s = 0.0;
    for (int p = 0; p < P; ++p) s += wp[p] * ((pose[r * P + p] - mean[r]) * (pose[c * P + p] - mean[c]));
    a.out[12 + tid] = s;
  }
  for (int p = tid; p < P; p += blockDim.x) a.out[48 + p] = wp[p];
}

}

hipError_t launch_init_particles(const double* init6xP, int P, const Pose0& pose, int mode, double* R, double* t,
                                 double* Rtot, double* pose_out, int refresh_pose, double* eul, hipStream_t st, const BeginZero* zero) {
  BeginZero z{};
  if (zero) z = *zero;
  unsigned int most = 0;
  for (int a = 0; a < z.n; ++a) most = z.dwords[a] > most ? z.dwords[a] : most;
  int blocks = (P + 127) / 128;
  const int for_zero = (int)((most + 128u * 32u - 1u) / (128u * 32u));
  if (for_zero > blocks) blocks = for_zero > 256 ? 256 : for_zero;
  hipLaunchKernelGGL(k_init_particles, dim3(blocks), dim3(128), 0, st, init6xP, P, pose, mode, R, t, Rtot,
                     pose_out, refresh_pose, eul, z);
  return hipGetLastError();
}

hipError_t launch_stats(const StatsArgs& a, hipStream_t st) {
  hipLaunchKernelGGL(k_stats, dim3(1), dim3(256), 0, st, a);
  return hipGetLastError();
}

hipError_t launch_stats_weighted(const StatsArgs& a, const double* w, hipStream_t st) {
  hipLaunchKernelGGL(k_stats_weighted, dim3(1), dim3(256), 0, st, a, w);
  return hipGetLastError();
}

}
```

### svn-icp_amd/csrc/registration_plan.hpp

```cpp
#pragma once
#include <cstddef>
#include <cstdint>
#include <initializer_list>

#include "stage_a_plan.hpp"

namespace svnicp {

struct Tuning {
  KnnOption knn;
  int knn_prefilter_mfma = 1;
  int fallback_sliced_max = -1;
  int accum = 3;
  int update_fused = 0;
  int fused_update_max_p = 128;
  int wgpcu_search = 0, wgpcu_accum = 0;
  int tp = 0;
  int accum_min_steps = 0;
  int group_stride = 0;
  int scan_split = 0;
  int debug = 0;
  int single_fused = 1;
  int small_chain = 1;
  int persistent = 0;
  int median_inline = -1;
  int brute_qb = 0;
  int sort_joint = 1;
  int table_select = 1;
  int full_corr = 0;
};

struct RegistrationFacts {
  int P = 0, K = 0, I = 0;
  int64_t B = 0, M = 0;
  bool svgd = false, check_early_stop = false, record_trace = false;
  bool profiling = false;
  bool shard_set = false;
  int p_lo = 0, p_hi = 0;
  int row_world = 1;
  int batch = 0;
  bool explicit_tab = false;
  int tab_I = 0;
  bool plane = false;
  bool normals_supplied = false;
  int normal_k = 16;
  int weighting = 0;
  int nshard() const { return p_hi - p_lo; }
  bool whole_shard() const { return p_lo == 0 && p_hi == P; }
};

constexpr int64_t kMinibatchMaxRows = 1ll << 22;
struct RegistrationRows {
  bool mb;
  int64_t Bq;
  int64_t Bt;
  int64_t Bi;
};
inline RegistrationRows registration_rows(int batch, int I, int64_t B) {
  if (batch == 0 || I <= 0) return {false, B, B, B};
  const int64_t n = (int64_t)I * batch;
  return {true, B < n ? B : n, n, batch};
}

struct Refusal { bool holds; const char* why; };
inline const char* first_refusal(std::initializer_list<Refusal> ladder) {
  for (const Refusal& r : ladder)
    if (r.holds) return r.why;
  return nullptr;
}
constexpr const char* kMinibatchRefusal = "svnicp_align: mini-batch mode (svnicp_set_minibatch) is not available here: ";
constexpr const char* kPlaneRefusal = "svnicp_align: the point-to-plane residual (svnicp_set_residual) is not available here: ";
constexpr const char* kWeightingRefusal = "svnicp_align: particle weighting (svnicp_set_particle_weighting) is not available here: ";
constexpr const char* kScoringRefusal = "svnicp_score_particles: the last registration cannot be scored: ";

inline const char* minibatch_refusal(const RegistrationFacts& f, const Tuning& t) {
  if (f.batch == 0) return nullptr;
  return first_refusal({
      {f.batch < 0, "batch_size must be positive"},
      {f.shard_set && !f.whole_shard(), "a partial particle shard (svnicp_set_shard) is set"},
      {f.row_world > 1, "a source-row shard (svnicp_set_row_shard) is set"},
      {t.full_corr != 0, "option correspondence=full is set"},
      {t.persistent != 0, "option chain=persistent is set"},
      {(int64_t)f.I * f.batch > kMinibatchMaxRows, "iterations * batch_size exceeds 2^22 table rows (about 2.5 KB of tables per row)"},
      {f.explicit_tab && f.tab_I != f.I, "the explicit index table's iteration count differs from params.iterations"},
  });
}
inline const char* plane_refusal(const RegistrationFacts& f, const Tuning& t) {
  if (!f.plane) return nullptr;
  return first_refusal({
      {f.svgd, "SVGD mode has no Hessian to put the plane residual in"},
      {f.shard_set && !f.whole_shard(), "a partial particle shard (svnicp_set_shard) is set"},
      {f.row_world > 1, "a source-row shard (svnicp_set_row_shard) is set: the rank exchange carries the 22 point-to-point sums"},
      {f.batch != 0, "mini-batch mode (svnicp_set_minibatch) is set"},
      {t.full_corr != 0, "option correspondence=full is set"},
      {t.persistent != 0, "option chain=persistent is set"},
      {t.accum != 3, "option accum is not split: the plane kernel consumes the search kernel's winner index"},
      {f.K > 128, "knn_count exceeds 128: the plane kernel consumes the matrix-pipe search kernel's winner index"},
      {!f.normals_supplied && f.M < f.normal_k, "the target has fewer points than normal_k and no normals were supplied"},
  });
}
inline const char* scoring_refusal(const RegistrationFacts& f, const Tuning& t) {
  return first_refusal({
      {f.shard_set && !f.whole_shard(), "a partial particle shard (svnicp_set_shard) is set"},
      {f.row_world > 1, "a source-row shard (svnicp_set_row_shard) is set: this context holds a part of the scan"},
      {f.batch != 0, "mini-batch mode (svnicp_set_minibatch) is set: its candidate tables are per drawn position"},
      {t.full_corr != 0, "option correspondence=full is set: the iterations did not search the candidate table"},
  });
}
inline const char* weighting_refusal(const RegistrationFacts& f, const Tuning& t) {
  if (f.weighting == 0) return nullptr;
  if (f.weighting != 1) return "unknown weighting kind";
  if (f.svgd) return "SVGD mode: the weight option belongs to SVNICP's constructor only";
  return scoring_refusal(f, t);
}
inline const char* full_corr_refusal(const RegistrationFacts& f, const Tuning& t, int variant, bool stage_a_k1) {
  if (!t.full_corr || f.nshard() <= 0) return nullptr;
  return first_refusal({
      {variant != 3, "correspondence = full needs the split stage B (accum = split, more than 8 particles or knn_count <= 128)"},
      {!stage_a_k1, "correspondence = full needs knn_count <= 128 (Morton-tile stage A) or knn = v1"},
  });
}

struct AccumPlan { int PW, WP, TP, grid_x, grid_y, tiles_per_block, Ppad, RS, f32, K, sgrid_x, pts_per_block, spts_per_block; int64_t n_tiles; size_t smem;
                   int small;  };
constexpr int kSmallChainBlocks = 32;

inline int stage_b_variant(int accum, int K, int nshard, bool full_corr, bool plane) {
  if (accum != 3) return accum;
  if (nshard <= 0 || K > 128 || (nshard <= 8 && !full_corr && !plane)) return 1;
  return 3;
}
inline AccumPlan stage_b_shape(int variant, int nshard, int K) {
  AccumPlan pl{};
  pl.f32 = variant;
  if (nshard <= 0) return pl;
  int PW = variant == 3 ? 16 : 8;
  while (PW < 64 && PW < nshard) PW <<= 1;
  int WP = 1;
  if (PW == 64) { WP = (nshard + 63) / 64; if (WP >= 3) WP = 4; }
  pl.PW = PW; pl.WP = WP; pl.K = K;
  pl.grid_y = (nshard + PW * WP - 1) / (PW * WP);
  pl.Ppad = pl.grid_y * PW * WP;
  pl.RS = (3 * K) | 1;
  return pl;
}
inline bool small_registration(const AccumPlan& shape, const RegistrationFacts& f, const Tuning& t, int64_t Bi) {
  return shape.f32 == 3 && shape.grid_y == 1 && Bi * f.nshard() <= (1 << 19) && t.small_chain && f.P >= 2 && f.P <= 128 &&
         f.P <= t.fused_update_max_p && !t.update_fused && f.row_world == 1 && f.whole_shard() && !t.full_corr && !f.plane;
}
inline AccumPlan plan_stage_b(const RegistrationFacts& f, const Tuning& t, int64_t Bi) {
  AccumPlan pl = stage_b_shape(stage_b_variant(t.accum, f.K, f.nshard(), t.full_corr != 0, f.plane), f.nshard(), f.K);
  pl.small = small_registration(pl, f, t, Bi) ? 1 : 0;
  return pl;
}

inline bool select_writes_table(const RegistrationFacts& f, const Tuning& t, const StageAPlan& a, const AccumPlan& b) {
  return t.table_select && a.kernel == KnnKernel::Tiles && a.K == f.K && b.f32 == 3 && f.batch == 0 && !f.shard_set;
}

inline bool joint_morton_sort(const RegistrationFacts& f, const Tuning& t, const StageAPlan& a) {
  return t.sort_joint && a.kernel == KnnKernel::Tiles && a.rows == f.B && f.batch == 0 && !f.shard_set;
}

enum class StepChain {
  OneKernel,
  SmallChain,
  InlineMedian,
  SideStream,
};
constexpr int kMedianInlineMaxP = 128;

struct StepPlan {
  StepChain chain = StepChain::OneKernel;
  bool single_fused = false;
};
inline StepPlan plan_step(const RegistrationFacts& f, const Tuning& t, const AccumPlan& pl) {
  StepPlan s;
  if (f.P < 2 || (t.update_fused && f.P <= t.fused_update_max_p)) s.chain = StepChain::OneKernel;
  else if (pl.small) s.chain = StepChain::SmallChain;
  else if (f.P <= kMedianInlineMaxP && f.P <= t.fused_update_max_p && t.median_inline != 0) s.chain = StepChain::InlineMedian;
  else s.chain = StepChain::SideStream;
  s.single_fused = f.P == 1 && !f.svgd && f.row_world == 1 && f.p_lo == 0 && f.p_hi == 1 && !t.full_corr && t.single_fused && pl.f32 == 1 &&
                   !f.plane;
  return s;
}

inline bool small_registration_supported(int PW, int WP, int K) {
  return K >= 97 && K <= 100 && ((WP == 1 && (PW == 16 || PW == 32 || PW == 64)) || (PW == 64 && WP == 2));
}

constexpr int kChunk = 4;
struct DrivePlan {
  bool persistent_try = false;
  bool defer_fin = false;
  bool follow = false;
};
inline DrivePlan plan_drive(const RegistrationFacts& f, const Tuning& t, const AccumPlan& pl, const StepPlan& s, bool blocking) {
  DrivePlan d;
  d.persistent_try = s.chain == StepChain::SmallChain && t.persistent && !f.record_trace && !f.profiling && f.I > 0 &&
                     small_registration_supported(pl.PW, pl.WP, f.K);
  d.defer_fin = f.check_early_stop && !f.record_trace && pl.f32 == 3 && !t.full_corr && s.chain != StepChain::OneKernel;
  d.follow = blocking && f.check_early_stop && f.I > 2 * kChunk;
  return d;
}

}
```

### svn-icp_amd/csrc/spatial_prep.hip

```cpp
#include <cstring>

#include <rocprim/device/device_radix_sort.hpp>

#include "kernels.hpp"

namespace svnicp {

namespace {

__device__ __forceinline__ unsigned long long enc_f64(double v) {
  const long long b = __double_as_longlong(v);
  return b < 0 ? ~(unsigned long long)b : ((unsigned long long)b | 0x8000000000000000ull);
}
__device__ __forceinline__ double dec_f64(unsigned long long e) {
  const unsigned long long b = (e & 0x8000000000000000ull) ? (e & 0x7fffffffffffffffull) : ~e;
  return __longlong_as_double((long long)b);
}
__device__ __forceinline__ float next_down(float f) {
  if (f == 0.0f) return -1.401298464e-45f;
  int b = __float_as_int(f);
  b += (f > 0.0f) ? -1 : 1;
  return __int_as_float(b);
}
__device__ __forceinline__ float next_up(float f) {
  if (f == 0.0f) return 1.401298464e-45f;
  int b = __float_as_int(f);
  b += (f > 0.0f) ? 1 : -1;
  return __int_as_float(b);
}
__device__ __forceinline__ float f32_floor(double v) { float f = (float)v; return ((double)f > v) ? next_down(f) : f; }
__device__ __forceinline__ float f32_ceil(double v) { float f = (float)v; return ((double)f < v) ? next_up(f) : f; }

__global__ __launch_bounds__(256) void k_bbox(const double* __restrict__ pts, int64_t n, unsigned long long* __restrict__ bbox) {
  double lo[3] = {__builtin_huge_val(), __builtin_huge_val(), __builtin_huge_val()};
  double hi[3] = {-__builtin_huge_val(), -__builtin_huge_val(), -__builtin_huge_val()};
  for (int64_t i = (int64_t)blockIdx.x * blockDim.x + threadIdx.x; i < n; i += (int64_t)gridDim.x * blockDim.x) {
#pragma unroll
    for (int d = 0; d < 3; ++d) { const double v = pts[3 * i + d]; lo[d] = fmin(lo[d], v); hi[d] = fmax(hi[d], v); }
  }
#pragma unroll
  for (int d = 0; d < 3; ++d) {
    for (int off = 32; off > 0; off >>= 1) {
      lo[d] = fmin(lo[d], __shfl_xor(lo[d], off, kWave));
      hi[d] = fmax(hi[d], __shfl_xor(hi[d], off, kWave));
    }
  }
  __shared__ double s_lo[4][3], s_hi[4][3];
  const int wave = threadIdx.x >> 6;
  if ((threadIdx.x & 63) == 0) {
#pragma unroll
    for (int d = 0; d < 3; ++d) { s_lo[wave][d] = lo[d]; s_hi[wave][d] = hi[d]; }
  }
  __syncthreads();
  if (threadIdx.x < 3) {
    const int d = threadIdx.x;
    double l = s_lo[0][d], h = s_hi[0][d];
    for (int w = 1; w < 4; ++w) { l = fmin(l, s_lo[w][d]); h = fmax(h, s_hi[w][d]); }
    if (l <= h) { atomicMin(&bbox[d], enc_f64(l)); atomicMax(&bbox[3 + d], enc_f64(h)); }
  }
}


__device__ __forceinline__ unsigned int spread10(unsigned int v) {
  v &= 0x3ffu;
  v = (v | (v << 16)) & 0x030000ffu;
  v = (v | (v << 8)) & 0x0300f00fu;
  v = (v | (v << 4)) & 0x030c30c3u;
  v = (v | (v << 2)) & 0x09249249u;
  return v;
}

__global__ void k_morton_keys(const double* __restrict__ pts, int64_t i0, int64_t n, int transform, Pose0 pose,
                              const unsigned long long* __restrict__ bbox, unsigned int* __restrict__ keys,
                              int32_t* __restrict__ vals, unsigned int key_or) {
  const int64_t e = (int64_t)blockIdx.x * blockDim.x + threadIdx.x;
  if (e >= n) return;
  const int64_t i = i0 + e;
  double p[3] = {pts[3 * i], pts[3 * i + 1], pts[3 * i + 2]};
  if (transform) {
    double x, y, z;
    stage_a_query(pose, p[0], p[1], p[2], &x, &y, &z);
    p[0] = x; p[1] = y; p[2] = z;
  }
  unsigned int c[3];
#pragma unroll
  for (int d = 0; d < 3; ++d) {
    const double lo = dec_f64(bbox[d]), hi = dec_f64(bbox[3 + d]);
    double u = (hi > lo) ? (p[d] - lo) / (hi - lo) : 0.0;
    if (!(u > 0.0)) u = 0.0;
    if (u > 0.999999) u = 0.999999;
    c[d] = (unsigned int)(u * 1024.0);
  }
  keys[e] = spread10(c[0]) | (spread10(c[1]) << 1) | (spread10(c[2]) << 2) | key_or;
  vals[e] = (int32_t)i;
}

__global__ __launch_bounds__(256) void k_targets_sorted(const double* __restrict__ tgt, int64_t M,
                                                        const int32_t* __restrict__ order, double* __restrict__ tx,
                                                        double* __restrict__ ty, double* __restrict__ tz,
                                                        float* __restrict__ txf, float* __restrict__ tyf,
                                                        float* __restrict__ tzf, int32_t* __restrict__ torig,
                                                        float* __restrict__ tile_box , int n_tiles,
                                                        unsigned long long* __restrict__ emax_bits,
                                                        float4* __restrict__ tile_a ,
                                                        float4* __restrict__ tile_o ) {
  __shared__ float red[4][6];
  __shared__ float s_org[3], s_c[4];
  __shared__ __align__(16) float s_rows[2048];
  const int tile = blockIdx.x;
  float lo[3] = {__builtin_huge_valf(), __builtin_huge_valf(), __builtin_huge_valf()};
  float hi[3] = {-__builtin_huge_valf(), -__builtin_huge_valf(), -__builtin_huge_valf()};
  double e = 0.0;
  double px[2], py[2], pz[2];
#pragma unroll
  for (int h = 0; h < 2; ++h) {
    const int r = threadIdx.x + 256 * h;
    const int64_t j = (int64_t)tile * 512 + r;
    const double nan = __builtin_nan("");
    double x = nan, y = nan, z = nan;
    int32_t o = 0;
    if (j < M) {
      o = order[j];
      x = tgt[3 * (int64_t)o]; y = tgt[3 * (int64_t)o + 1]; z = tgt[3 * (int64_t)o + 2];
      const double m = fmax(fabs(x), fmax(fabs(y), fabs(z)));
      e = fmax(e, (m == m) ? m : __builtin_huge_val());
      if (x == x) { lo[0] = __builtin_fminf(lo[0], f32_floor(x)); hi[0] = __builtin_fmaxf(hi[0], f32_ceil(x)); }
      if (y == y) { lo[1] = __builtin_fminf(lo[1], f32_floor(y)); hi[1] = __builtin_fmaxf(hi[1], f32_ceil(y)); }
      if (z == z) { lo[2] = __builtin_fminf(lo[2], f32_floor(z)); hi[2] = __builtin_fmaxf(hi[2], f32_ceil(z)); }
    }
    tx[j] = x; ty[j] = y; tz[j] = z;
    txf[j] = (float)x; tyf[j] = (float)y; tzf[j] = (float)z;
    torig[j] = o;
    px[h] = x; py[h] = y; pz[h] = z;
  }
  for (int off = 32; off > 0; off >>= 1) {
#pragma unroll
    for (int d = 0; d < 3; ++d) {
      lo[d] = __builtin_fminf(lo[d], __shfl_xor(lo[d], off, kWave));
      hi[d] = __builtin_fmaxf(hi[d], __shfl_xor(hi[d], off, kWave));
    }
    e = fmax(e, __shfl_xor(e, off, kWave));
  }
  const int wave = threadIdx.x >> 6, lane = threadIdx.x & 63;
  if (lane == 0) {
#pragma unroll
    for (int d = 0; d < 3; ++d) { red[wave][d] = lo[d]; red[wave][3 + d] = hi[d]; }
    if (e > 0.0) atomicMax(emax_bits, (unsigned long long)__double_as_longlong(e));
  }
  __syncthreads();
  if (threadIdx.x < 6) {
    const int d = threadIdx.x;
    float v = red[0][d];
    for (int w = 1; w < 4; ++w) v = d < 3 ? __builtin_fminf(v, red[w][d]) : __builtin_fmaxf(v, red[w][d]);
    tile_box[(size_t)d * n_tiles + tile] = v;
    red[0][d] = v;
  }
  __syncthreads();
  if (threadIdx.x < 3) {
    const int d = threadIdx.x;
    const float c = (float)(0.5 * ((double)red[0][d] + (double)red[0][3 + d]));
    s_org[d] = (c - c == 0.0f) ? c : 0.0f;
  }
  __syncthreads();
  const float o0 = s_org[0], o1 = s_org[1], o2 = s_org[2];
  float cmax = 0.0f;
#pragma unroll
  for (int h = 0; h < 2; ++h) {
    const int r = threadIdx.x + 256 * h;
    const int64_t j = (int64_t)tile * 512 + r;
    float v[4] = {0.0f, 0.0f, 0.0f, 1e30f};
    if (j < M) {
      v[0] = (float)(px[h] - (double)o0); v[1] = (float)(py[h] - (double)o1); v[2] = (float)(pz[h] - (double)o2);
      const double n2 = ((double)v[0] * (double)v[0] + (double)v[1] * (double)v[1]) + (double)v[2] * (double)v[2];
      v[3] = (float)n2;
      const float n = next_up(f32_ceil(sqrt(n2)));
      cmax = (n - n == 0.0f) ? __builtin_fmaxf(cmax, n) : __builtin_huge_valf();
    }
    const int rb = r >> 4, mj = r & 15;
#pragma unroll
    for (int c = 0; c < 4; ++c) s_rows[(((rb >> 2) * 64) + c * 16 + mj) * 4 + (rb & 3)] = v[c];
  }
  for (int off = 32; off > 0; off >>= 1) cmax = __builtin_fmaxf(cmax, __shfl_xor(cmax, off, kWave));
  if (lane == 0) s_c[wave] = cmax;
  __syncthreads();
  const float4* rows4 = reinterpret_cast<const float4*>(s_rows);
  tile_a[(size_t)tile * 512 + threadIdx.x] = rows4[threadIdx.x];
  tile_a[(size_t)tile * 512 + 256 + threadIdx.x] = rows4[256 + threadIdx.x];
  if (threadIdx.x == 0)
    tile_o[tile] = make_float4(o0, o1, o2, __builtin_fmaxf(__builtin_fmaxf(s_c[0], s_c[1]), __builtin_fmaxf(s_c[2], s_c[3])));
}

}

size_t sort_temp_bytes(size_t n, int key_bits) {
  size_t bytes = 0;
  (void)rocprim::radix_sort_pairs(nullptr, bytes, (unsigned int*)nullptr, (unsigned int*)nullptr, (int32_t*)nullptr,
                                  (int32_t*)nullptr, n, 0, key_bits, (hipStream_t)0);
  return bytes;
}

hipError_t launch_morton_order(const double* pts, int64_t i0, int64_t n, int transform, const Pose0& pose,
                               const unsigned long long* bbox, unsigned int* keys_a, unsigned int* keys_b,
                               int32_t* vals_a, int32_t* order, void* temp, size_t temp_bytes, hipStream_t st) {
  if (n <= 0) return hipSuccess;
  hipLaunchKernelGGL(k_morton_keys, dim3((unsigned)((n + 255) / 256)), dim3(256), 0, st, pts, i0, n, transform, pose, bbox,
                     keys_a, vals_a, 0u);
  hipError_t e = hipGetLastError();
  if (e != hipSuccess) return e;
  return rocprim::radix_sort_pairs(temp, temp_bytes, keys_a, keys_b, vals_a, order, (size_t)n, 0, 30, st);
}

hipError_t launch_morton_order_joint(const double* tgt, int64_t M, const double* qsrc, int64_t n, const Pose0& pose,
                                     const unsigned long long* bbox, unsigned int* keys_a, unsigned int* keys_b,
                                     int32_t* vals_a, int32_t* order, void* temp, size_t temp_bytes, hipStream_t st) {
  if (M <= 0 || n <= 0) return hipErrorInvalidValue;
  hipLaunchKernelGGL(k_morton_keys, dim3((unsigned)((M + 255) / 256)), dim3(256), 0, st, tgt, 0, M, 0, pose, bbox, keys_a, vals_a, 0u);
  hipLaunchKernelGGL(k_morton_keys, dim3((unsigned)((n + 255) / 256)), dim3(256), 0, st, qsrc, 0, n, 1, pose, bbox, keys_a + M,
                     vals_a + M, 1u << 30);
  hipError_t e = hipGetLastError();
  if (e != hipSuccess) return e;
  return rocprim::radix_sort_pairs(temp, temp_bytes, keys_a, keys_b, vals_a, order, (size_t)(M + n), 0, 31, st);
}

hipError_t launch_bbox(const double* pts, int64_t n, unsigned long long* bbox, hipStream_t st) {
  hipError_t e = hipMemsetAsync(bbox, 0xff, 3 * sizeof(unsigned long long), st);
  if (e != hipSuccess) return e;
  e = hipMemsetAsync(bbox + 3, 0, 3 * sizeof(unsigned long long), st);
  if (e != hipSuccess) return e;
  int64_t nb = (n + 255) / 256;
  if (nb > 256) nb = 256;
  hipLaunchKernelGGL(k_bbox, dim3((unsigned)nb), dim3(256), 0, st, pts, n, bbox);
  return hipGetLastError();
}

hipError_t launch_targets_sorted(const double* tgt, int64_t M, int64_t Mp, const int32_t* order, double* tx, double* ty,
                                 double* tz, float* txf, float* tyf, float* tzf, int32_t* torig, float* tile_box,
                                 unsigned long long* emax_bits, float4* tile_a, float4* tile_o, hipStream_t st) {
  hipError_t e = hipMemsetAsync(emax_bits, 0, sizeof(unsigned long long), st);
  if (e != hipSuccess) return e;
  const int n_tiles = (int)(Mp / 512);
  hipLaunchKernelGGL(k_targets_sorted, dim3(n_tiles), dim3(256), 0, st, tgt, M, order, tx, ty, tz, txf, tyf, tzf, torig,
                     tile_box, n_tiles, emax_bits, tile_a, tile_o);
  return hipGetLastError();
}

}
```

### svn-icp_amd/csrc/stage_a_host.hpp

```cpp
#pragma once
#include <algorithm>
#include <cstdio>
#include <initializer_list>
#include <vector>

#include "device_buffer.hpp"
#include "kernels.hpp"

namespace svnicp_host {
using namespace svnicp;

struct StageAEnv {
  hipStream_t stream;
  const Tuning& tune;
  int num_cus;
  bool record_trace;
  const double* tgt;
  int64_t B, M;
  const Pose0& pose0;
};

struct TableOut { float4* rows; double* anchor; float* cmax; };

struct StageA {
  StageAPlan plan;
  bool writes_table = false;
  TargetLayout held = TargetLayout::None;
  bool layout_pending = false;
  DevBuf<double> tx, ty, tz;
  DevBuf<float> txf, tyf, tzf, tile_box;
  DevBuf<float4> tile_a, tile_o;
  DevBuf<int32_t> torig;
  DevBuf<unsigned long long> emax, bbox;
  DevBuf<double> cand_d2;
  DevBuf<int32_t> cand_idx;
  DevBuf<double> pool_d, sl_d, fail_tau, qrec;
  DevBuf<int32_t> pool_i, sl_i, pool2, fail_list, stat_n;
  DevBuf<int> fail_count;
  DevBuf<int> stage_fail_count;
  DevBuf<int32_t> stage_fail_list;
  bool stage_kept = false;
  DevBuf<unsigned int> keys_a, keys_b;
  DevBuf<int32_t> vals_a, order_t, qorder;
  DevBuf<unsigned char> sort_tmp;
  size_t sort_n = 0, sort_tmp_bytes = 0;
  int sort_bits = 0;
  DevBuf<int32_t> arena, chunk_tab;
  DevBuf<unsigned long long> dbg_phase;
  static constexpr size_t kDbgPhaseWaves = 65536;

  static StageAPlan plan_for(const StageAEnv& e, int64_t rows, int K) { return plan_stage_a(rows, e.M, K, e.tune.knn, e.tune.fallback_sliced_max); }
  template <class Obj>
  int begin(Obj* o, const StageAEnv& e, int64_t rows, int K, std::initializer_list<int> Ks, bool joint_sort = false) {
    plan = plan_for(e, rows, K);
    stage_kept = false;
    layout_pending = false;
    const size_t Bq = (size_t)rows, B = (size_t)e.B, M = (size_t)e.M, Mp = (size_t)plan.Mp;
    size_t S = 0, slice_entries = 0;
    for (const int k : Ks) { S = std::max<size_t>(S, knn_pool_size(k)); slice_entries = std::max<size_t>(slice_entries, (size_t)knn_slice_count(k) * k); }
    HIPCHK(o, cand_idx.ensure(Bq * K));
    HIPCHK(o, cand_d2.ensure(Bq * K));
    if (plan.kernel == KnnKernel::Stream) {
      HIPCHK(o, pool_d.ensure(Bq * S)); HIPCHK(o, pool_i.ensure(Bq * S));
    } else {
      HIPCHK(o, fail_count.ensure(1));
    }
    if (plan.has_fallback()) {
      if (plan.kernel == KnnKernel::Tiles) {
        HIPCHK(o, pool2.ensure(Bq * kTilesBase));
        HIPCHK(o, arena.ensure((size_t)plan.arena_cap * kTilesChunk));
        HIPCHK(o, chunk_tab.ensure(tiles_chunk_tab_words(rows)));
        if (e.record_trace) HIPCHK(o, stat_n.ensure(B));
      } else {
        HIPCHK(o, pool2.ensure(Bq * plan.S2));
      }
      HIPCHK(o, fail_list.ensure(Bq)); HIPCHK(o, fail_tau.ensure(Bq));
      HIPCHK(o, qrec.ensure(Bq * 6));
      HIPCHK(o, pool_d.ensure((size_t)kFallbackGrid * 4 * kFallbackQW * S));
      HIPCHK(o, pool_i.ensure((size_t)kFallbackGrid * 4 * kFallbackQW * S));
      if (plan.sliced_max > 0) { HIPCHK(o, sl_d.ensure((size_t)plan.sliced_max * slice_entries)); HIPCHK(o, sl_i.ensure((size_t)plan.sliced_max * slice_entries)); }
      if (e.tune.full_corr) { HIPCHK(o, stage_fail_count.ensure(1)); HIPCHK(o, stage_fail_list.ensure(B)); }
    }
    if (plan.layout == TargetLayout::None) return SVNICP_OK;
    HIPCHK(o, tx.ensure(Mp)); HIPCHK(o, ty.ensure(Mp)); HIPCHK(o, tz.ensure(Mp));
    HIPCHK(o, txf.ensure(Mp)); HIPCHK(o, tyf.ensure(Mp)); HIPCHK(o, tzf.ensure(Mp));
    HIPCHK(o, torig.ensure(Mp)); HIPCHK(o, emax.ensure(1));
    if (plan.layout == TargetLayout::Morton) {
      const bool joint = joint_sort && held != plan.layout;
      const size_t nmax = joint ? M + B : std::max(M, B);
      const int bits = joint ? 31 : 30;
      HIPCHK(o, keys_a.ensure(nmax)); HIPCHK(o, keys_b.ensure(nmax)); HIPCHK(o, vals_a.ensure(nmax));
      HIPCHK(o, order_t.ensure(joint ? M + B : M)); HIPCHK(o, qorder.ensure(B));
      HIPCHK(o, bbox.ensure(6)); HIPCHK(o, tile_box.ensure(6 * (Mp / kTileSlots)));
      HIPCHK(o, tile_a.ensure(Mp)); HIPCHK(o, tile_o.ensure(Mp / kTileSlots));
      if (nmax > sort_n || bits > sort_bits) {
        sort_n = std::max(sort_n, nmax); sort_bits = std::max(sort_bits, bits);
        sort_tmp_bytes = std::max(sort_temp_bytes(sort_n, sort_bits), sort_temp_bytes(sort_n, 30));
        HIPCHK(o, sort_tmp.ensure(sort_tmp_bytes));
      }
      if (joint) { layout_pending = true; return SVNICP_OK; }
    }
    return ensure_layout(o, e);
  }

  template <class Obj>
  int ensure_layout(Obj* o, const StageAEnv& e) {
    layout_pending = false;
    if (held == plan.layout || plan.layout == TargetLayout::None) return SVNICP_OK;
    if (plan.layout == TargetLayout::Hashed) {
      HIPCHK(o, launch_targets_soa2(e.tgt, e.M, plan.Mp, tx.p, ty.p, tz.p, txf.p, tyf.p, tzf.p, torig.p, emax.p, e.stream));
    } else {
      HIPCHK(o, launch_bbox(e.tgt, e.M, bbox.p, e.stream));
      HIPCHK(o, launch_morton_order(e.tgt, 0, e.M, 0, e.pose0, bbox.p, keys_a.p, keys_b.p, vals_a.p, order_t.p, sort_tmp.p, sort_tmp_bytes, e.stream));
      HIPCHK(o, launch_targets_sorted(e.tgt, e.M, plan.Mp, order_t.p, tx.p, ty.p, tz.p, txf.p, tyf.p, tzf.p, torig.p, tile_box.p, emax.p, tile_a.p, tile_o.p, e.stream));
    }
    held = plan.layout;
    return SVNICP_OK;
  }

  hipError_t launch_fallback(KnnArgs a, hipStream_t stream) {
    a.qlist = fail_list.p; a.qlist_count = fail_count.p; a.list_grid = kFallbackGrid; a.list_qw = kFallbackQW;
    a.slice_max_queries = plan.sliced_max; a.slices = 0;
    hipError_t e = launch_knn_topk(a, stream);
    if (e != hipSuccess || plan.sliced_max <= 0) return e;
    a.slices = knn_slice_count(a.K);
    a.merge_n = 1;
    while (a.merge_n < a.slices * a.K) a.merge_n <<= 1;
    a.sl_d = sl_d.p; a.sl_i = sl_i.p;
    e = launch_knn_topk(a, stream);
    if (e != hipSuccess) return e;
    return launch_knn_merge_slices(a, stream);
  }

  template <class Obj>
  int clear_dbg_phase(Obj* o, hipStream_t stream, size_t waves) {
    HIPCHK(o, dbg_phase.ensure(8 + 8 * kDbgPhaseWaves));
    HIPCHK(o, hipMemsetAsync(dbg_phase.p, 0, (8 + 8 * waves) * sizeof(unsigned long long), stream));
    return SVNICP_OK;
  }

  template <class Obj>
  int print_phases(Obj* o, const StageAEnv& e, int64_t n, size_t dbg_waves) {
    std::vector<unsigned long long> h(8 + 8 * dbg_waves);
    HIPCHK(o, hipMemcpyAsync(h.data(), dbg_phase.p, h.size() * sizeof(unsigned long long), hipMemcpyDeviceToHost, e.stream));
    HIPCHK(o, hipStreamSynchronize(e.stream));
    if (plan.kernel == KnnKernel::Brute) {
      const int qb = e.tune.brute_qb > 0 ? e.tune.brute_qb : knn_brute_queries_per_block(n, e.num_cus);
      const double nwg = (double)((n + qb - 1) / qb);
      fprintf(stderr, "[svnicp] k_knn_brute (%d queries per workgroup) thread-0 cycles per workgroup: pass A %.0f, bound %.0f, pass B %.0f, general path %.0f, rank + write %.0f\n",
              qb, h[0] / nwg, h[1] / nwg, h[2] / nwg, h[3] / nwg, h[4] / nwg);
      return SVNICP_OK;
    }
    fprintf(stderr, "[svnicp] k_knn_tiles wave cycles: rank %llu seed %llu scan %llu barrier waits + hand-over %llu | counts: seed tiles %llu scan tiles %llu scan (query, tile) pairs %llu\n", h[0], h[1], h[2], h[3], h[4], h[5], h[6]);
    auto column = [&](const char* tag, int col, unsigned long long floor_) {
      std::vector<unsigned long long> v;
      for (size_t w = 0; w < dbg_waves; ++w) { const unsigned long long x = h[8 + 8 * w + col]; if (x >= floor_) v.push_back(x); }
      if (v.empty()) return;
      std::sort(v.begin(), v.end());
      fprintf(stderr, "[svnicp]   seed kernel %-12s n %6zu  p50 %8llu  p90 %8llu  p99 %8llu  max %8llu cycles\n", tag, v.size(), v[v.size() / 2],
              v[v.size() * 9 / 10], v[v.size() * 99 / 100], v.back());
    };
    column("rank", 0, 5000); column("seed", 1, 1); column("tile loop", 5, 1); column("bisection", 6, 1); column("waits", 3, 0);
    return SVNICP_OK;
  }

  template <class Obj>
  int search(Obj* o, const StageAEnv& e, const double* qsrc, const Pose0& pose, int K, int32_t* out_idx, double* out_d2, int64_t b_lo,
             int64_t b_hi, const TableOut* tbl = nullptr, bool whole_source = false) {
    const int64_t n = b_hi - b_lo;
    const bool joint = layout_pending && whole_source && plan.kernel == KnnKernel::Tiles && b_lo == 0 && n == e.B && n > 0;
    if (layout_pending && !joint)
      if (const int rc = ensure_layout(o, e)) return rc;
    KnnArgs a{};
    a.src = qsrc; a.pose = pose; a.tx = tx.p; a.ty = ty.p; a.tz = tz.p; a.torig = torig.p;
    a.M = e.M; a.Mp = plan.Mp; a.b_lo = b_lo; a.b_hi = b_hi; a.K = K; a.S = knn_pool_size(K);
    a.pool_d = pool_d.p; a.pool_i = pool_i.p; a.out_idx = out_idx; a.out_d2 = out_d2;
    switch (plan.kernel) {
    case KnnKernel::Brute: {
      KnnBruteArgs k{};
      k.src = qsrc; k.pose = pose; k.tgt = e.tgt; k.M = e.M; k.b_lo = b_lo; k.b_hi = b_hi; k.K = K; k.out_idx = out_idx; k.out_d2 = out_d2;
      if (e.tune.debug) {
        if (const int rc = clear_dbg_phase(o, e.stream, 0)) return rc;
        k.phase_cycles = dbg_phase.p;
      }
      HIPCHK(o, launch_knn_brute(k, e.num_cus, e.tune.brute_qb, e.stream));
      if (e.tune.debug) return print_phases(o, e, n, 0);
      return SVNICP_OK;
    }
    case KnnKernel::Tiles: {
      if (n <= 0) return SVNICP_OK;
      const int32_t* qord = qorder.p + b_lo;
      if (joint) {
        HIPCHK(o, launch_bbox(e.tgt, e.M, bbox.p, e.stream));
        HIPCHK(o, launch_morton_order_joint(e.tgt, e.M, qsrc, n, pose, bbox.p, keys_a.p, keys_b.p, vals_a.p, order_t.p, sort_tmp.p, sort_tmp_bytes, e.stream));
        HIPCHK(o, launch_targets_sorted(e.tgt, e.M, plan.Mp, order_t.p, tx.p, ty.p, tz.p, txf.p, tyf.p, tzf.p, torig.p, tile_box.p, emax.p, tile_a.p, tile_o.p, e.stream));
        held = plan.layout; layout_pending = false;
        qord = order_t.p + e.M;
      } else {
        HIPCHK(o, launch_morton_order(qsrc, b_lo, n, 1, pose, bbox.p, keys_a.p, keys_b.p, vals_a.p, qorder.p + b_lo, sort_tmp.p, sort_tmp_bytes, e.stream));
      }
      KnnTilesArgs k{};
      k.src = qsrc; k.pose = pose; k.qorder = qord;
      k.tx = tx.p; k.ty = ty.p; k.tz = tz.p; k.txf = txf.p; k.tyf = tyf.p; k.tzf = tzf.p;
      k.torig = torig.p; k.tile_box = tile_box.p; k.emax_bits = emax.p;
      k.tile_a = tile_a.p; k.tile_o = tile_o.p; k.prefilter_mfma = e.tune.knn_prefilter_mfma;
      k.M = e.M; k.Mp = plan.Mp; k.n_tiles = (int)(plan.Mp / kTileSlots); k.b_lo = b_lo; k.b_hi = b_hi; k.K = K; k.S2 = plan.S2;
      k.pool = pool2.p; k.out_idx = out_idx; k.out_d2 = tbl ? nullptr : out_d2;
      k.tgt = e.tgt;
      if (tbl) { k.tbl_a = tbl->rows; k.tbl_anchor = tbl->anchor; k.tbl_cmax = tbl->cmax; }
      k.arena = arena.p; k.chunk_tab = chunk_tab.p; k.arena_cap = plan.arena_cap; k.tab_rows = plan.rows;
      k.scan_split = e.tune.scan_split == 4 ? 4 : 8;
      {
        const unsigned int ng = (unsigned int)((n + 63) / 64);
        unsigned int st = e.tune.group_stride > 0 ? (unsigned int)e.tune.group_stride : 17u;
        auto gcd = [](unsigned int x, unsigned int y) { while (y) { const unsigned int t = x % y; x = y; y = t; } return x; };
        while (st > 1 && gcd(st, ng) != 1) st += 2;
        if (ng <= 2 || st >= ng) st = 1;
        k.group_stride = st;
      }
      HIPCHK(o, hipMemsetAsync(chunk_tab.p, 0xff, tiles_chunk_tab_words(plan.rows) * sizeof(int32_t), e.stream));
      k.fail_list = fail_list.p; k.fail_count = fail_count.p; k.fail_tau = fail_tau.p; k.qrec = qrec.p;
      a.qthr = fail_tau.p;
      if (e.record_trace) k.stat_n = stat_n.p;
      HIPCHK(o, hipMemsetAsync(fail_count.p, 0, sizeof(int), e.stream));
      const size_t dbg_waves = (size_t)((n + 63) / 64) * 4;
      const bool dbg = e.tune.debug && dbg_waves <= kDbgPhaseWaves;
      if (dbg) {
        if (const int rc = clear_dbg_phase(o, e.stream, dbg_waves)) return rc;
        k.phase_cycles = dbg_phase.p;
      }
      HIPCHK(o, launch_knn_tiles(k, e.stream));
      if (dbg)
        if (const int rc = print_phases(o, e, n, dbg_waves)) return rc;
      HIPCHK(o, launch_fallback(a, e.stream));
      if (tbl)
        HIPCHK(o, launch_build_table3_list(out_idx, fail_list.p, fail_count.p, e.B, K, e.tgt, e.M, tbl->anchor, tbl->rows, tbl->cmax, e.stream));
      return SVNICP_OK;
    }
    case KnnKernel::SeededScan: {
      KnnScanArgs k{};
      k.src = qsrc; k.pose = pose; k.tx = tx.p; k.ty = ty.p; k.tz = tz.p;
      k.txf = txf.p; k.tyf = tyf.p; k.tzf = tzf.p; k.torig = torig.p; k.emax_bits = emax.p;
      k.M = e.M; k.Mp = plan.Mp; k.Ms = plan.scan_Ms; k.b_lo = b_lo; k.b_hi = b_hi; k.K = K; k.S2 = plan.S2;
      k.seed_rank = plan.scan_rank; k.pool = pool2.p; k.out_idx = out_idx; k.out_d2 = out_d2;
      k.fail_list = fail_list.p; k.fail_count = fail_count.p;
      HIPCHK(o, hipMemsetAsync(fail_count.p, 0, sizeof(int), e.stream));
      HIPCHK(o, launch_knn_scan(k, e.stream));
      HIPCHK(o, launch_fallback(a, e.stream));
      return SVNICP_OK;
    }
    case KnnKernel::Stream:
      HIPCHK(o, launch_knn_topk(a, e.stream));
    }
    return SVNICP_OK;
  }

  int64_t block_rows(int64_t n) const { return std::max<int64_t>(1, std::min<int64_t>(plan.rows, n)); }
  template <class Obj, class Done = int (*)(int64_t, int64_t)>
  int search_blocks(Obj* o, const StageAEnv& e, const double* q, int64_t n, int Kq, int32_t* out_idx, double* out_d2, int out_step,
                    Done done = [](int64_t, int64_t) { return 0; }) {
    Pose0 ident{};
    ident.R0[0] = ident.R0[4] = ident.R0[8] = 1.0;
    const int64_t rows = block_rows(n);
    for (int64_t lo = 0; lo < n; lo += rows) {
      const int64_t cnt = std::min<int64_t>(rows, n - lo), off = lo * out_step * Kq;
      if (const int rc = search(o, e, q + 3 * lo, ident, Kq, out_idx + off, out_d2 + off, 0, cnt)) return rc;
      if (const int rc = done(lo, cnt)) return rc;
    }
    return SVNICP_OK;
  }

  template <class Obj>
  int keep_stage_fallbacks(Obj* o, const StageAEnv& e) {
    if (!plan.has_fallback()) return SVNICP_OK;
    HIPCHK(o, stage_fail_count.ensure(1)); HIPCHK(o, stage_fail_list.ensure((size_t)plan.rows));
    HIPCHK(o, hipMemcpyAsync(stage_fail_count.p, fail_count.p, sizeof(int), hipMemcpyDeviceToDevice, e.stream));
    HIPCHK(o, hipMemcpyAsync(stage_fail_list.p, fail_list.p, (size_t)plan.rows * sizeof(int32_t), hipMemcpyDeviceToDevice, e.stream));
    stage_kept = true;
    return SVNICP_OK;
  }
  const int* fallback_count() const {
    if (plan.kernel == KnnKernel::Stream) return nullptr;
    return stage_kept ? stage_fail_count.p : fail_count.p;
  }
  const int32_t* fallback_rows() const { return stage_kept ? stage_fail_list.p : fail_list.p; }
  const int32_t* survivors(bool record_trace) const { return plan.kernel == KnnKernel::Tiles && record_trace ? stat_n.p : nullptr; }
};

}
```

Before: 150.9 registrations/s.

## Replace rocprim radix sort with custom segmented LSD sort and fold memsets into kernels

Adds a custom 10-bit-digit LSD radix sort (histogram plus scatter kernels) that sorts the target and query key segments jointly and is meant to replace the rocprim radix sort used for Morton ordering. The chunk table 0xff fill moves into the Morton key kernel, and the bbox, emax and fail_count initialisations move into the particle init kernel, which removes several small hipMemsetAsync launches per registration. It also adds a sort_kernel tuning option and a test driver build. The risks are in correctness of the custom sort's stability and segment handling, and in the stateful start_words_set flag that must stay correctly synchronised with the layout_pending state.

```diff
diff --git a/__graft_entry__.py b/__graft_entry__.py
--- a/__graft_entry__.py
+++ b/__graft_entry__.py
@@ -38,6 +38,7 @@
     if os.path.isdir("/root/reference"):
         subprocess.check_call(["make", "-C", os.path.join(ROOT, "oracle"), "ref"])
     build_cpp_host()
+    build_morton_order_driver()
     pkg = load_package()
     pkg.load_library()
 
@@ -52,6 +53,18 @@
     subprocess.check_call(["/opt/rocm/bin/hipcc", "-std=c++17", "-O2", "-Wall", "-Werror", "-I", os.path.join(ROOT, "include"), "-I", host,
                            os.path.join(host, "sharded_drive.cpp"), "-L", PKG_DIR, "-lsvnicp_hip", "-lrccl",
                            "-Wl,-rpath,$ORIGIN/..", "-o", exe])
+    return exe
+
+
+def build_morton_order_driver() -> str:
+    csrc = os.path.join(PKG_DIR, "csrc")
+    exe = os.path.join(ROOT, "tests", "morton_order_driver")
+    srcs = [os.path.join(ROOT, "tests", "morton_order_driver.hip")] + [os.path.join(csrc, f) for f in (
+        "spatial_prep.hip", "kernels.hpp", "device_math.hpp", "registration_plan.hpp", "stage_a_plan.hpp")]
+    if os.path.exists(exe) and all(os.path.getmtime(exe) >= os.path.getmtime(f) for f in srcs):
+        return exe
+    subprocess.check_call(["/opt/rocm/bin/hipcc", "-O3", "-std=c++17", "--offload-arch=gfx950", "-ffp-contract=off", "-Wall", "-Wno-unused-function",
+                           "-I", csrc, srcs[0], srcs[1], "-o", exe])
     return exe
 
 
diff --git a/svn-icp_amd/csrc/api.hip b/svn-icp_amd/csrc/api.hip
--- a/svn-icp_amd/csrc/api.hip
+++ b/svn-icp_amd/csrc/api.hip
@@ -299,7 +299,7 @@
 int svnicp_set_source(svnicp_ctx* c, const double* src, int64_t B, int mem_kind) {
   CTX_CHECK(c);
   if (!src || B < 1) return fail(c, SVNICP_ERR_INVALID, "svnicp_set_source: need B >= 1");
-  if (B > 0x7fffffffLL) return fail(c, SVNICP_ERR_INVALID, "svnicp_set_source: cloud too large");
+  if (const char* why = cloud_rows_refusal(B)) return fail(c, SVNICP_ERR_INVALID, std::string("svnicp_set_source: ") + why);
   if (const int rc = upload_cloud(c, c->cloud.src, src, B, mem_kind)) return rc;
   c->B = B;
   c->cloud.src_set = true;
@@ -309,7 +309,7 @@
 int svnicp_set_target(svnicp_ctx* c, const double* tgt, int64_t M, int mem_kind) {
   CTX_CHECK(c);
   if (!tgt || M < 1) return fail(c, SVNICP_ERR_INVALID, "svnicp_set_target: need M >= 1");
-  if (M > 0x7fffffffLL) return fail(c, SVNICP_ERR_INVALID, "svnicp_set_target: cloud too large");
+  if (const char* why = cloud_rows_refusal(M)) return fail(c, SVNICP_ERR_INVALID, std::string("svnicp_set_target: ") + why);
   if (const int rc = upload_cloud(c, c->cloud.tgt, tgt, M, mem_kind)) return rc;
   c->M = M;
   c->sa.held = TargetLayout::None;
@@ -321,7 +321,7 @@
 int svnicp_set_clouds(svnicp_ctx* c, const double* src, int64_t B, const double* tgt, int64_t M, int mem_kind) {
   CTX_CHECK(c);
   if (!src || !tgt || B < 1 || M < 1) return fail(c, SVNICP_ERR_INVALID, "svnicp_set_clouds: need B >= 1, M >= 1");
-  if (M > 0x7fffffffLL || B > 0x7fffffffLL) return fail(c, SVNICP_ERR_INVALID, "svnicp_set_clouds: cloud too large");
+  if (const char* why = cloud_rows_refusal(M > B ? M : B)) return fail(c, SVNICP_ERR_INVALID, std::string("svnicp_set_clouds: ") + why);
   if (const int rc = svnicp_set_source(c, src, B, mem_kind)) return rc;
   return svnicp_set_target(c, tgt, M, mem_kind);
 }
@@ -414,6 +414,7 @@
                            else if (v == "general") { t.small_chain = 0; t.persistent = 0; } else ok = false; }
   else if (k == "median") { if (v == "auto") t.median_inline = -1; else if (v == "stream") t.median_inline = 0; else if (v == "inline") t.median_inline = 1; else ok = false; }
   else if (k == "sort") { if (v == "joint") t.sort_joint = 1; else if (v == "separate") t.sort_joint = 0; else ok = false; }
+  else if (k == "sort_kernel") { if (v == "radix") t.sort_merge = 0; else if (v == "merge") t.sort_merge = 1; else ok = false; }
   else if (k == "table") { if (v == "select") t.table_select = 1; else if (v == "gather") t.table_select = 0; else ok = false; }
   else if (k == "correspondence") { if (v == "fast") t.full_corr = 0; else if (v == "full") t.full_corr = 1; else ok = false; }
   else return fail(c, SVNICP_ERR_INVALID, "svnicp_set_option: unknown option '" + k + "'");
@@ -527,9 +528,15 @@
     HIPCHK(c, c->st.small_bar.ensure(8));
     add(c->st.small_bar.p, 8 * sizeof(unsigned int));
     if (c->prm.mode == SVNICP_MODE_SVGD) add(c->st.opt.p, (size_t)P * 18 * sizeof(double));
+    const bool sa_words = c->sa.layout_pending;
+    if (sa_words) {
+      add(c->sa.bbox.p + 3, 3 * sizeof(unsigned long long)); add(c->sa.emax.p, sizeof(unsigned long long)); add(c->sa.fail_count.p, sizeof(int));
+      z.ones = reinterpret_cast<unsigned int*>(c->sa.bbox.p); z.ones_dwords = 6;
+    }
     z.ctl = c->st.ctl.p; z.iterations = I;
     HIPCHK(c, launch_init_particles(c->st.init_pose.p, P, c->pose0, 2, c->st.R.p, c->st.t.p, c->st.Rtot.p, c->st.pose_out.p, 0,
                                     nullptr, c->stream, &z));
+    c->sa.start_words_set = sa_words;
   }
   if (c->mb.batch > 0 && !c->mb.explicit_tab) {
     c->mb.base = minibatch_stream_base(c->mb.seed, c->mb.n);
diff --git a/svn-icp_amd/csrc/kernels.hpp b/svn-icp_amd/csrc/kernels.hpp
--- a/svn-icp_amd/csrc/kernels.hpp
+++ b/svn-icp_amd/csrc/kernels.hpp
@@ -104,16 +104,18 @@
 hipError_t launch_candidate_dist2(const double* src, const Pose0& pose, const double* tgt, int64_t M, const int32_t* idx, int64_t B, int K,
                                   double* d2, hipStream_t st);
 size_t sort_temp_bytes(size_t n, int key_bits);
-hipError_t launch_bbox(const double* pts, int64_t n, unsigned long long* bbox, hipStream_t st);
+hipError_t launch_bbox(const double* pts, int64_t n, unsigned long long* bbox, bool cleared, hipStream_t st);
 hipError_t launch_morton_order(const double* pts, int64_t i0, int64_t n, int transform, const Pose0& pose,
                                const unsigned long long* bbox, unsigned int* keys_a, unsigned int* keys_b,
-                               int32_t* vals_a, int32_t* order, void* temp, size_t temp_bytes, hipStream_t st);
+                               int32_t* vals_a, int32_t* order, void* temp, size_t temp_bytes, bool rocprim_sort, int32_t* fill_ff,
+                               size_t fill_words, hipStream_t st);
 hipError_t launch_morton_order_joint(const double* tgt, int64_t M, const double* qsrc, int64_t n, const Pose0& pose,
                                      const unsigned long long* bbox, unsigned int* keys_a, unsigned int* keys_b,
-                                     int32_t* vals_a, int32_t* order, void* temp, size_t temp_bytes, hipStream_t st);
+                                     int32_t* vals_a, int32_t* order, void* temp, size_t temp_bytes, bool rocprim_sort, int32_t* fill_ff,
+                                     size_t fill_words, hipStream_t st);
 hipError_t launch_targets_sorted(const double* tgt, int64_t M, int64_t Mp, const int32_t* order, double* tx, double* ty,
                                  double* tz, float* txf, float* tyf, float* tzf, int32_t* torig, float* tile_box,
-                                 unsigned long long* emax_bits, float4* tile_a, float4* tile_o, hipStream_t st);
+                                 unsigned long long* emax_bits, bool emax_cleared, float4* tile_a, float4* tile_o, hipStream_t st);
 
 struct AccumArgs {
   const double* src;
@@ -190,7 +192,7 @@
   const double* plane_Hb;
 };
 size_t update_workspace_doubles(int P);
-struct BeginZero { unsigned int* ptr[6]; unsigned int dwords[6]; int n; int* ctl; int iterations; };
+struct BeginZero { unsigned int* ptr[10]; unsigned int dwords[10]; int n; int* ctl; int iterations; unsigned int* ones; unsigned int ones_dwords; };
 hipError_t launch_init_particles(const double* init6xP, int P, const Pose0& pose, int mode, double* R, double* t,
                                  double* Rtot, double* pose_out, int refresh_pose, double* eul, hipStream_t st, const BeginZero* zero = nullptr);
 int single_particle_grid(int64_t B);
diff --git a/svn-icp_amd/csrc/particle_state.hip b/svn-icp_amd/csrc/particle_state.hip
--- a/svn-icp_amd/csrc/particle_state.hip
+++ b/svn-icp_amd/csrc/particle_state.hip
@@ -9,6 +9,7 @@
   const int p = blockIdx.x * blockDim.x + threadIdx.x;
   for (int a = 0; a < z.n; ++a)
     for (unsigned int e = (unsigned int)p; e < z.dwords[a]; e += gridDim.x * blockDim.x) z.ptr[a][e] = 0u;
+  for (unsigned int e = (unsigned int)p; e < z.ones_dwords; e += gridDim.x * blockDim.x) z.ones[e] = 0xffffffffu;
   if (z.ctl && p == 0) { z.ctl[0] = 0; z.ctl[1] = z.iterations; z.ctl[2] = 0; z.ctl[3] = 0; }
   if (p >= P) return;
   double r[3] = {0, 0, 0}, tv[3], Rm[9];
diff --git a/svn-icp_amd/csrc/registration_plan.hpp b/svn-icp_amd/csrc/registration_plan.hpp
--- a/svn-icp_amd/csrc/registration_plan.hpp
+++ b/svn-icp_amd/csrc/registration_plan.hpp
@@ -26,6 +26,7 @@
   int median_inline = -1;
   int brute_qb = 0;
   int sort_joint = 1;
+  int sort_merge = 0;
   int table_select = 1;
   int full_corr = 0;
 };
@@ -73,6 +74,9 @@
 constexpr const char* kWeightingRefusal = "svnicp_align: particle weighting (svnicp_set_particle_weighting) is not available here: ";
 constexpr const char* kScoringRefusal = "svnicp_score_particles: the last registration cannot be scored: ";
 
+constexpr int64_t kMaxCloudRows = 0x7fffffffLL;
+inline const char* cloud_rows_refusal(int64_t rows) { return rows > kMaxCloudRows ? "cloud too large" : nullptr; }
+
 inline const char* minibatch_refusal(const RegistrationFacts& f, const Tuning& t) {
   if (f.batch == 0) return nullptr;
   return first_refusal({
diff --git a/svn-icp_amd/csrc/spatial_prep.hip b/svn-icp_amd/csrc/spatial_prep.hip
--- a/svn-icp_amd/csrc/spatial_prep.hip
+++ b/svn-icp_amd/csrc/spatial_prep.hip
@@ -72,8 +72,9 @@
 
 __global__ void k_morton_keys(const double* __restrict__ pts, int64_t i0, int64_t n, int transform, Pose0 pose,
                               const unsigned long long* __restrict__ bbox, unsigned int* __restrict__ keys,
-                              int32_t* __restrict__ vals, unsigned int key_or) {
+                              int32_t* __restrict__ vals, unsigned int key_or, int32_t* __restrict__ fill_ff, size_t fill_words) {
   const int64_t e = (int64_t)blockIdx.x * blockDim.x + threadIdx.x;
+  for (size_t w = (size_t)e; w < fill_words; w += (size_t)gridDim.x * blockDim.x) fill_ff[w] = -1;
   if (e >= n) return;
   const int64_t i = i0 + e;
   double p[3] = {pts[3 * i], pts[3 * i + 1], pts[3 * i + 2]};
@@ -190,43 +191,199 @@
     tile_o[tile] = make_float4(o0, o1, o2, __builtin_fmaxf(__builtin_fmaxf(s_c[0], s_c[1]), __builtin_fmaxf(s_c[2], s_c[3])));
 }
 
+#ifndef SVNICP_SORT_ITEMS
+#define SVNICP_SORT_ITEMS 4
+#endif
+constexpr int kSortThreads = 1024, kSortItems = SVNICP_SORT_ITEMS, kSortWaves = kSortThreads / kWave;
+constexpr int kSortBlockItems = kSortThreads * kSortItems;
+constexpr int kSortBits = 10, kSortBins = 1 << kSortBits;
+constexpr int kSortMaxBlocks = 512;
+static_assert(kSortBins == kSortThreads, "k_sort_scatter: thread t owns digit t");
+
+struct SortSegs { unsigned int n0, n1; int nb0; };
+struct SortBlock { unsigned int lo, n, first; int b0, b1; };
+__device__ __forceinline__ SortBlock sort_block(const SortSegs& s) {
+  SortBlock k;
+  const int b = (int)blockIdx.x;
+  if (b < s.nb0) { k.lo = 0u; k.n = s.n0; k.b0 = 0; k.b1 = s.nb0; }
+  else { k.lo = s.n0; k.n = s.n1; k.b0 = s.nb0; k.b1 = (int)gridDim.x; }
+  k.first = k.lo + (unsigned int)(b - k.b0) * (unsigned int)kSortBlockItems;
+  return k;
+}
+
+__device__ __forceinline__ unsigned long long digit_peers(unsigned int d, unsigned long long live) {
+  unsigned long long m = live;
+#pragma unroll
+  for (int k = 0; k < kSortBits; ++k) {
+    const unsigned int bit = (d >> k) & 1u;
+    m &= __ballot(bit) ^ ((unsigned long long)bit - 1ull);
+  }
+  return m;
+}
+
+__global__ __launch_bounds__(kSortThreads) void k_sort_hist(const unsigned int* __restrict__ keys, SortSegs segs, int shift,
+                                                            unsigned int* __restrict__ hist ) {
+  __shared__ unsigned int h[kSortBins];
+  h[threadIdx.x] = 0u;
+  __syncthreads();
+  const SortBlock blk = sort_block(segs);
+  const int lane = threadIdx.x & (kWave - 1);
+  const unsigned int base = blk.first + (threadIdx.x >> 6) * (unsigned int)(kWave * kSortItems) + lane;
+  unsigned int key[kSortItems];
+#pragma unroll
+  for (int r = 0; r < kSortItems; ++r) {
+    const unsigned int i = base + r * kWave;
+    key[r] = i - blk.lo < blk.n ? keys[i] : 0u;
+  }
+#pragma unroll
+  for (int r = 0; r < kSortItems; ++r) {
+    const bool live = base + r * kWave - blk.lo < blk.n;
+    const unsigned int d = (key[r] >> shift) & (kSortBins - 1);
+    const unsigned int d0 = (unsigned int)__builtin_amdgcn_readfirstlane((int)d);
+    if (__all(live && d == d0)) {
+      if (lane == 0) atomicAdd(&h[d0], (unsigned int)kWave);
+    } else if (live) {
+      atomicAdd(&h[d], 1u);
+    }
+  }
+  __syncthreads();
+  hist[(size_t)blockIdx.x * kSortBins + threadIdx.x] = h[threadIdx.x];
+}
+
+__global__ __launch_bounds__(kSortThreads) void k_sort_scatter(const unsigned int* __restrict__ keys_in, const int32_t* __restrict__ vals_in,
+                                                               unsigned int* __restrict__ keys_out , int32_t* __restrict__ vals_out,
+                                                               SortSegs segs, int shift, const unsigned int* __restrict__ hist) {
+  __shared__ unsigned short cnt[kSortWaves][kSortBins];
+  __shared__ unsigned int off[kSortBins];
+  __shared__ unsigned int wsum[kSortWaves];
+  const int tid = threadIdx.x, lane = tid & (kWave - 1), wave = tid >> 6;
+  for (int w = 0; w < kSortWaves; ++w) cnt[w][tid] = 0;
+  __syncthreads();
+  const SortBlock blk = sort_block(segs);
+  volatile unsigned short* mine = cnt[wave];
+  const unsigned int base = blk.first + wave * (unsigned int)(kWave * kSortItems) + lane;
+  const unsigned long long lt = (1ull << lane) - 1ull;
+  unsigned int key[kSortItems];
+  int32_t val[kSortItems];
+  unsigned short rank[kSortItems];
+#pragma unroll
+  for (int r = 0; r < kSortItems; ++r) {
+    const unsigned int i = base + r * kWave;
+    const bool live = i - blk.lo < blk.n;
+    key[r] = live ? keys_in[i] : 0u;
+    val[r] = live ? vals_in[i] : 0;
+  }
+#pragma unroll
+  for (int r = 0; r < kSortItems; ++r) {
+    const bool live = base + r * kWave - blk.lo < blk.n;
+    const unsigned int d = (key[r] >> shift) & (kSortBins - 1);
+    const unsigned long long m = digit_peers(d, __ballot(live));
+    const unsigned int prior = mine[d];
+    rank[r] = (unsigned short)(prior + (unsigned int)__popcll(m & lt));
+    if (live && lane == __ffsll((long long)m) - 1) mine[d] = (unsigned short)(prior + (unsigned int)__popcll(m));
+  }
+  __syncthreads();
+  unsigned int tot = 0u, pre = 0u;
+  for (int b = blk.b0; b < blk.b1; ++b) {
+    const unsigned int v = hist[(size_t)b * kSortBins + tid];
+    tot += v;
+    pre += b < (int)blockIdx.x ? v : 0u;
+  }
+  unsigned int inc = tot;
+  for (int o = 1; o < kWave; o <<= 1) { const unsigned int x = __shfl_up(inc, o, kWave); if (lane >= o) inc += x; }
+  if (lane == kWave - 1) wsum[wave] = inc;
+  __syncthreads();
+  unsigned int start = inc - tot;
+  for (int w = 0; w < wave; ++w) start += wsum[w];
+  off[tid] = start + pre;
+  unsigned int run = 0u;
+  for (int w = 0; w < kSortWaves; ++w) { const unsigned int c = cnt[w][tid]; cnt[w][tid] = (unsigned short)run; run += c; }
+  __syncthreads();
+#pragma unroll
+  for (int r = 0; r < kSortItems; ++r) {
+    const bool live = base + r * kWave - blk.lo < blk.n;
+    const unsigned int d = (key[r] >> shift) & (kSortBins - 1);
+    const unsigned int dst = off[d] + cnt[wave][d] + rank[r];
+    if (live && dst < blk.n) {
+      if (keys_out) keys_out[blk.lo + dst] = key[r];
+      vals_out[blk.lo + dst] = val[r];
+    }
+  }
+}
+
+size_t lsd_sort_blocks(size_t n) { return (n + kSortBlockItems - 1) / kSortBlockItems; }
+size_t lsd_sort_temp_bytes(size_t n) { return (lsd_sort_blocks(n) + 1) * kSortBins * sizeof(unsigned int); }
+bool lsd_sort_serves(size_t n0, size_t n1, size_t temp_bytes) {
+  return n0 > 0 && lsd_sort_blocks(n0) + lsd_sort_blocks(n1) <= (size_t)kSortMaxBlocks && temp_bytes >= lsd_sort_temp_bytes(n0 + n1);
+}
+
+hipError_t lsd_sort_pass(const unsigned int* keys_in, const int32_t* vals_in, unsigned int* keys_out, int32_t* vals_out, const SortSegs& segs, int nb,
+                         int shift, unsigned int* hist, hipStream_t st) {
+  hipLaunchKernelGGL(k_sort_hist, dim3(nb), dim3(kSortThreads), 0, st, keys_in, segs, shift, hist);
+  hipLaunchKernelGGL(k_sort_scatter, dim3(nb), dim3(kSortThreads), 0, st, keys_in, vals_in, keys_out, vals_out, segs, shift, (const unsigned int*)hist);
+  return hipGetLastError();
+}
+
+hipError_t lsd_sort_pairs(unsigned int* keys_a, unsigned int* keys_b, int32_t* vals_a, int32_t* order, size_t n0, size_t n1, void* temp,
+                          hipStream_t st) {
+  unsigned int* hist = static_cast<unsigned int*>(temp);
+  const SortSegs segs{(unsigned int)n0, (unsigned int)n1, (int)lsd_sort_blocks(n0)};
+  const int nb = segs.nb0 + (int)lsd_sort_blocks(n1);
+  hipError_t e = lsd_sort_pass(keys_a, vals_a, keys_b, order, segs, nb, 0, hist, st);
+  if (e != hipSuccess) return e;
+  e = lsd_sort_pass(keys_b, order, keys_a, vals_a, segs, nb, kSortBits, hist, st);
+  if (e != hipSuccess) return e;
+  return lsd_sort_pass(keys_a, vals_a, nullptr, order, segs, nb, 2 * kSortBits, hist, st);
+}
+
+hipError_t sort_pairs(bool rocprim_sort, unsigned int* keys_a, unsigned int* keys_b, int32_t* vals_a, int32_t* order, size_t n0, size_t n1,
+                      void* temp, size_t temp_bytes, hipStream_t st) {
+  if (!rocprim_sort && lsd_sort_serves(n0, n1, temp_bytes)) return lsd_sort_pairs(keys_a, keys_b, vals_a, order, n0, n1, temp, st);
+  return rocprim::radix_sort_pairs(temp, temp_bytes, keys_a, keys_b, vals_a, order, n0 + n1, 0, n1 ? 31 : 30, st);
+}
+
 }
 
 size_t sort_temp_bytes(size_t n, int key_bits) {
   size_t bytes = 0;
   (void)rocprim::radix_sort_pairs(nullptr, bytes, (unsigned int*)nullptr, (unsigned int*)nullptr, (int32_t*)nullptr,
                                   (int32_t*)nullptr, n, 0, key_bits, (hipStream_t)0);
-  return bytes;
+  return bytes > lsd_sort_temp_bytes(n) ? bytes : lsd_sort_temp_bytes(n);
 }
 
 hipError_t launch_morton_order(const double* pts, int64_t i0, int64_t n, int transform, const Pose0& pose,
                                const unsigned long long* bbox, unsigned int* keys_a, unsigned int* keys_b,
-                               int32_t* vals_a, int32_t* order, void* temp, size_t temp_bytes, hipStream_t st) {
-  if (n <= 0) return hipSuccess;
+                               int32_t* vals_a, int32_t* order, void* temp, size_t temp_bytes, bool rocprim_sort, int32_t* fill_ff,
+                               size_t fill_words, hipStream_t st) {
+  if (n <= 0) return fill_words ? hipMemsetAsync(fill_ff, 0xff, fill_words * sizeof(int32_t), st) : hipSuccess;
   hipLaunchKernelGGL(k_morton_keys, dim3((unsigned)((n + 255) / 256)), dim3(256), 0, st, pts, i0, n, transform, pose, bbox,
-                     keys_a, vals_a, 0u);
+                     keys_a, vals_a, 0u, fill_ff, fill_words);
   hipError_t e = hipGetLastError();
   if (e != hipSuccess) return e;
-  return rocprim::radix_sort_pairs(temp, temp_bytes, keys_a, keys_b, vals_a, order, (size_t)n, 0, 30, st);
+  return sort_pairs(rocprim_sort, keys_a, keys_b, vals_a, order, (size_t)n, 0, temp, temp_bytes, st);
 }
 
 hipError_t launch_morton_order_joint(const double* tgt, int64_t M, const double* qsrc, int64_t n, const Pose0& pose,
                                      const unsigned long long* bbox, unsigned int* keys_a, unsigned int* keys_b,
-                                     int32_t* vals_a, int32_t* order, void* temp, size_t temp_bytes, hipStream_t st) {
+                                     int32_t* vals_a, int32_t* order, void* temp, size_t temp_bytes, bool rocprim_sort, int32_t* fill_ff,
+                                     size_t fill_words, hipStream_t st) {
   if (M <= 0 || n <= 0) return hipErrorInvalidValue;
-  hipLaunchKernelGGL(k_morton_keys, dim3((unsigned)((M + 255) / 256)), dim3(256), 0, st, tgt, 0, M, 0, pose, bbox, keys_a, vals_a, 0u);
+  hipLaunchKernelGGL(k_morton_keys, dim3((unsigned)((M + 255) / 256)), dim3(256), 0, st, tgt, 0, M, 0, pose, bbox, keys_a, vals_a, 0u,
+                     (int32_t*)nullptr, (size_t)0);
   hipLaunchKernelGGL(k_morton_keys, dim3((unsigned)((n + 255) / 256)), dim3(256), 0, st, qsrc, 0, n, 1, pose, bbox, keys_a + M,
-                     vals_a + M, 1u << 30);
+                     vals_a + M, 1u << 30, fill_ff, fill_words);
   hipError_t e = hipGetLastError();
   if (e != hipSuccess) return e;
-  return rocprim::radix_sort_pairs(temp, temp_bytes, keys_a, keys_b, vals_a, order, (size_t)(M + n), 0, 31, st);
-}
-
-hipError_t launch_bbox(const double* pts, int64_t n, unsigned long long* bbox, hipStream_t st) {
-  hipError_t e = hipMemsetAsync(bbox, 0xff, 3 * sizeof(unsigned long long), st);
-  if (e != hipSuccess) return e;
-  e = hipMemsetAsync(bbox + 3, 0, 3 * sizeof(unsigned long long), st);
-  if (e != hipSuccess) return e;
+  return sort_pairs(rocprim_sort, keys_a, keys_b, vals_a, order, (size_t)M, (size_t)n, temp, temp_bytes, st);
+}
+
+hipError_t launch_bbox(const double* pts, int64_t n, unsigned long long* bbox, bool cleared, hipStream_t st) {
+  if (!cleared) {
+    hipError_t e = hipMemsetAsync(bbox, 0xff, 3 * sizeof(unsigned long long), st);
+    if (e != hipSuccess) return e;
+    e = hipMemsetAsync(bbox + 3, 0, 3 * sizeof(unsigned long long), st);
+    if (e != hipSuccess) return e;
+  }
   int64_t nb = (n + 255) / 256;
   if (nb > 256) nb = 256;
   hipLaunchKernelGGL(k_bbox, dim3((unsigned)nb), dim3(256), 0, st, pts, n, bbox);
@@ -235,9 +392,11 @@
 
 hipError_t launch_targets_sorted(const double* tgt, int64_t M, int64_t Mp, const int32_t* order, double* tx, double* ty,
                                  double* tz, float* txf, float* tyf, float* tzf, int32_t* torig, float* tile_box,
-                                 unsigned long long* emax_bits, float4* tile_a, float4* tile_o, hipStream_t st) {
-  hipError_t e = hipMemsetAsync(emax_bits, 0, sizeof(unsigned long long), st);
-  if (e != hipSuccess) return e;
+                                 unsigned long long* emax_bits, bool emax_cleared, float4* tile_a, float4* tile_o, hipStream_t st) {
+  if (!emax_cleared) {
+    hipError_t e = hipMemsetAsync(emax_bits, 0, sizeof(unsigned long long), st);
+    if (e != hipSuccess) return e;
+  }
   const int n_tiles = (int)(Mp / 512);
   hipLaunchKernelGGL(k_targets_sorted, dim3(n_tiles), dim3(256), 0, st, tgt, M, order, tx, ty, tz, txf, tyf, tzf, torig,
                      tile_box, n_tiles, emax_bits, tile_a, tile_o);
diff --git a/svn-icp_amd/csrc/stage_a_host.hpp b/svn-icp_amd/csrc/stage_a_host.hpp
--- a/svn-icp_amd/csrc/stage_a_host.hpp
+++ b/svn-icp_amd/csrc/stage_a_host.hpp
@@ -27,6 +27,7 @@
   bool writes_table = false;
   TargetLayout held = TargetLayout::None;
   bool layout_pending = false;
+  bool start_words_set = false;
   DevBuf<double> tx, ty, tz;
   DevBuf<float> txf, tyf, tzf, tile_box;
   DevBuf<float4> tile_a, tile_o;
@@ -55,6 +56,7 @@
     plan = plan_for(e, rows, K);
     stage_kept = false;
     layout_pending = false;
+    start_words_set = false;
     const size_t Bq = (size_t)rows, B = (size_t)e.B, M = (size_t)e.M, Mp = (size_t)plan.Mp;
     size_t S = 0, slice_entries = 0;
     for (const int k : Ks) { S = std::max<size_t>(S, knn_pool_size(k)); slice_entries = std::max<size_t>(slice_entries, (size_t)knn_slice_count(k) * k); }
@@ -106,13 +108,15 @@
   template <class Obj>
   int ensure_layout(Obj* o, const StageAEnv& e) {
     layout_pending = false;
+    start_words_set = false;
     if (held == plan.layout || plan.layout == TargetLayout::None) return SVNICP_OK;
     if (plan.layout == TargetLayout::Hashed) {
       HIPCHK(o, launch_targets_soa2(e.tgt, e.M, plan.Mp, tx.p, ty.p, tz.p, txf.p, tyf.p, tzf.p, torig.p, emax.p, e.stream));
     } else {
-      HIPCHK(o, launch_bbox(e.tgt, e.M, bbox.p, e.stream));
-      HIPCHK(o, launch_morton_order(e.tgt, 0, e.M, 0, e.pose0, bbox.p, keys_a.p, keys_b.p, vals_a.p, order_t.p, sort_tmp.p, sort_tmp_bytes, e.stream));
-      HIPCHK(o, launch_targets_sorted(e.tgt, e.M, plan.Mp, order_t.p, tx.p, ty.p, tz.p, txf.p, tyf.p, tzf.p, torig.p, tile_box.p, emax.p, tile_a.p, tile_o.p, e.stream));
+      HIPCHK(o, launch_bbox(e.tgt, e.M, bbox.p, false, e.stream));
+      HIPCHK(o, launch_morton_order(e.tgt, 0, e.M, 0, e.pose0, bbox.p, keys_a.p, keys_b.p, vals_a.p, order_t.p, sort_tmp.p, sort_tmp_bytes,
+                                    e.tune.sort_merge != 0, nullptr, 0, e.stream));
+      HIPCHK(o, launch_targets_sorted(e.tgt, e.M, plan.Mp, order_t.p, tx.p, ty.p, tz.p, txf.p, tyf.p, tzf.p, torig.p, tile_box.p, emax.p, false, tile_a.p, tile_o.p, e.stream));
     }
     held = plan.layout;
     return SVNICP_OK;
@@ -171,6 +175,8 @@
     const bool joint = layout_pending && whole_source && plan.kernel == KnnKernel::Tiles && b_lo == 0 && n == e.B && n > 0;
     if (layout_pending && !joint)
       if (const int rc = ensure_layout(o, e)) return rc;
+    const bool words_set = start_words_set && joint;
+    start_words_set = false;
     KnnArgs a{};
     a.src = qsrc; a.pose = pose; a.tx = tx.p; a.ty = ty.p; a.tz = tz.p; a.torig = torig.p;
     a.M = e.M; a.Mp = plan.Mp; a.b_lo = b_lo; a.b_hi = b_hi; a.K = K; a.S = knn_pool_size(K);
@@ -190,14 +196,17 @@
     case KnnKernel::Tiles: {
       if (n <= 0) return SVNICP_OK;
       const int32_t* qord = qorder.p + b_lo;
+      const size_t tab_words = tiles_chunk_tab_words(plan.rows);
       if (joint) {
-        HIPCHK(o, launch_bbox(e.tgt, e.M, bbox.p, e.stream));
-        HIPCHK(o, launch_morton_order_joint(e.tgt, e.M, qsrc, n, pose, bbox.p, keys_a.p, keys_b.p, vals_a.p, order_t.p, sort_tmp.p, sort_tmp_bytes, e.stream));
-        HIPCHK(o, launch_targets_sorted(e.tgt, e.M, plan.Mp, order_t.p, tx.p, ty.p, tz.p, txf.p, tyf.p, tzf.p, torig.p, tile_box.p, emax.p, tile_a.p, tile_o.p, e.stream));
+        HIPCHK(o, launch_bbox(e.tgt, e.M, bbox.p, words_set, e.stream));
+        HIPCHK(o, launch_morton_order_joint(e.tgt, e.M, qsrc, n, pose, bbox.p, keys_a.p, keys_b.p, vals_a.p, order_t.p, sort_tmp.p, sort_tmp_bytes,
+                                            e.tune.sort_merge != 0, chunk_tab.p, tab_words, e.stream));
+        HIPCHK(o, launch_targets_sorted(e.tgt, e.M, plan.Mp, order_t.p, tx.p, ty.p, tz.p, txf.p, tyf.p, tzf.p, torig.p, tile_box.p, emax.p, words_set, tile_a.p, tile_o.p, e.stream));
         held = plan.layout; layout_pending = false;
         qord = order_t.p + e.M;
       } else {
-        HIPCHK(o, launch_morton_order(qsrc, b_lo, n, 1, pose, bbox.p, keys_a.p, keys_b.p, vals_a.p, qorder.p + b_lo, sort_tmp.p, sort_tmp_bytes, e.stream));
+        HIPCHK(o, launch_morton_order(qsrc, b_lo, n, 1, pose, bbox.p, keys_a.p, keys_b.p, vals_a.p, qorder.p + b_lo, sort_tmp.p, sort_tmp_bytes,
+                                      e.tune.sort_merge != 0, chunk_tab.p, tab_words, e.stream));
       }
       KnnTilesArgs k{};
       k.src = qsrc; k.pose = pose; k.qorder = qord;
@@ -218,11 +227,10 @@
         if (ng <= 2 || st >= ng) st = 1;
         k.group_stride = st;
       }
-      HIPCHK(o, hipMemsetAsync(chunk_tab.p, 0xff, tiles_chunk_tab_words(plan.rows) * sizeof(int32_t), e.stream));
       k.fail_list = fail_list.p; k.fail_count = fail_count.p; k.fail_tau = fail_tau.p; k.qrec = qrec.p;
       a.qthr = fail_tau.p;
       if (e.record_trace) k.stat_n = stat_n.p;
-      HIPCHK(o, hipMemsetAsync(fail_count.p, 0, sizeof(int), e.stream));
+      if (!words_set) HIPCHK(o, hipMemsetAsync(fail_count.p, 0, sizeof(int), e.stream));
       const size_t dbg_waves = (size_t)((n + 63) / 64) * 4;
       const bool dbg = e.tune.debug && dbg_waves <= kDbgPhaseWaves;
       if (dbg) {
```

New measurement: 152.6 registrations/s (median of 6 runs). 1.01x the previous value.
